# hbaatz/nerf-tex

Measured on AMD Instinct MI355X. Metric: ray-samples/sec (MLP+composite) at 800x800x64, higher is better.
Workload: dtype f32; 1 GPU; carpet 800x800x64: 640000 all-hit rays x 64 samples per GPU (BASELINE configs[1]), ParamNerf n_parameters=[1, 6], seeded glorot weights, inputs resident in HBM, fused PE+MLP+composite; rays_per_gpu=640000, hit_rays_total=640000, samples_per_ray=64

## Files before the change

nerf_tex_amd/csrc/ntx_backend_chain.hip:

```cpp
#include <algorithm>
#include <cstdio>
#include <cstdlib>
#include "ntx_trainer.h"
#include "ntx_train_device.h"
#include "ntx_encode.h"
namespace ntx_train {
enum { PACK_HIDDEN = 0, PACK_LINEAR = 1, PACK_AUX_ROW = 2, PACK_AUX_RGB = 3, PACK_COPY = 4 };
struct PackSeg {
    const float *src; long long sk, sc;
    int mode;
    int K, ncols, nt;
    float *dst; long long first, count;
};
struct PackArgs { const PackSeg *seg; int n_seg; long long total; };
__global__ void pack_kernel(PackArgs a) {
    const long long e = (long long)blockIdx.x * blockDim.x + threadIdx.x;
    if (e >= a.total) return;
    int lo = 0, hi = a.n_seg - 1;
    while (lo < hi) { const int mid = (lo + hi + 1) >> 1; if (a.seg[mid].first <= e) lo = mid; else hi = mid - 1; }
    const PackSeg &p = a.seg[lo];
    const long long o = e - p.first;
    float v = 0.0f;
    if (p.mode == PACK_COPY) v = p.src[o];
    else if (p.mode == PACK_AUX_ROW) {
        const int h = (int)(o >> 7) & 1, V = (int)(o & 127), k = hidden_row(V, h);
        v = k < p.K ? p.src[k * p.sk] : 0.0f;
    } else if (p.mode == PACK_AUX_RGB) {
        const int c = (int)(o >> 7), h = (int)(o >> 6) & 1, V = (int)(o & 63);
        v = p.src[hidden_row(V, h) * 3 + c];
    } else {
        const int c = (int)(o & 3), lane = (int)((o >> 2) & 63);
        const long long rec = o >> 8;
        const int G = p.nt / 4, g = (int)(rec % G), s = (int)(rec / G);
        const int f = lane & 31, kh = lane >> 5;
        const int k = p.mode == PACK_HIDDEN ? hidden_row(s, kh) : 2 * s + kh, col = 32 * (4 * g + c) + f;
        if (k < p.K && col < p.ncols) v = p.src[k * p.sk + col * p.sc];
    }
    p.dst[o] = v;
}

struct EncodeArgs {
    StepRays r;
    float *posO; int ptiles;
    float *dirO; int dtiles;
    float *dists;
};
template <bool IPE>
__global__ __launch_bounds__(64) void encode_kernel(EncodeArgs args) {
    const StepRays &a = args.r;
    const int lane = threadIdx.x, n = lane & 31, h = lane >> 5, blk = blockIdx.x, part = blockIdx.y;
    const long long m = (long long)blk * 32 + n;
    const bool valid = m < a.M();
    const int ray = valid ? (int)(m / a.S) : 0, s = valid ? (int)(m - (long long)ray * a.S) : 0;
    const int P = a.n_geo + a.n_app;
    const RayCtx rc = ray_ctx(a.rays_d, a.params, a.rays_per_param_row, ray, IPE ? P + 1 : P);
    const float *zray = a.z + (size_t)ray * (IPE ? a.S + 1 : a.S);
    const float e0 = zray[s], e1 = IPE ? zray[s + 1] : 0.0f;
    bool hit;
    const float z = depth_of(e0, hit);
    if (IPE) hit = hit && isfinite(e1);
    auto param = [&](int c) { return IPE ? spliced_param(rc.pr, c, a.blur_idx) : blurred_param(rc.pr, c, a.blur_idx, hit, a.cone, ray, z); };
    float *O = part == 0 ? args.posO : args.dirO;
    const int tiles = part == 0 ? args.ptiles : args.dtiles;
    auto put = [&](int row, float v) { O[o_index(blk, tiles, row, n)] = valid ? v : 0.0f; };
    auto fourier = [&](int r0, int D, int L, auto x) {
        if (h == 0) for (int c = 0; c < D; ++c) put(r0 + c, x(c));
        for (int f = 0; f < L; ++f)
            for (int c = 0; c < D; ++c) put(r0 + fourier_row_of(D, f, h, c), fourier_value(x(c), f, h));
    };
    if (part == 0) {
        int geo0;
        if (IPE) {
            float mean[3] = {a.rays_o[3 * ray], a.rays_o[3 * ray + 1], a.rays_o[3 * ray + 2]}, cov[3] = {0.0f, 0.0f, 0.0f};
            if (hit) {
                float t_mean, t_var, r_var;
                ntx::cone_moments((e0 + e1) / 2.0f, (e1 - e0) / 2.0f, rc.pr[a.blur_idx] * a.cone[ray], t_mean, t_var, r_var);
                for (int c = 0; c < 3; ++c) mean[c] = mean[c] + rc.d[c] * t_mean;
                ntx::cone_cov(t_var, r_var, rc.d, cov);
            }
            const int L = a.pos_freq;
            for (int f = 0; f < L; ++f)
                for (int c = 0; c < 3; ++c)
                    put(h * 3 * L + 3 * f + c, ntx::sin_q(mean[c] * ldexpf(1.0f, f), h) * expf(-0.5f * (cov[c] * ldexpf(1.0f, 2 * f))));
            geo0 = 6 * L;
        } else {
            const float o[3] = {a.rays_o[3 * ray], a.rays_o[3 * ray + 1], a.rays_o[3 * ray + 2]};
            fourier(0, 3, a.pos_freq, [&](int c) { return rc.point(o[c], c, z); });
            geo0 = fourier_width(3, a.pos_freq);
        }
        if (a.n_geo > 0) fourier(geo0, a.n_geo, a.param_freq, [&](int c) { return param(c); });
    } else {
        fourier(0, 3, a.dir_freq, [&](int c) { return rc.dir(c); });
        if (a.n_app > 0) fourier(fourier_width(3, a.dir_freq), a.n_app, a.param_freq, [&](int c) { return param(a.n_geo + c); });
        if (valid && h == 0) args.dists[(size_t)ray * a.S + s] = IPE ? segment_dist(e0, e1, hit, rc.dn) : sample_dist(zray, s, a.S, z, hit, rc.dn);
    }
}

struct EncodeSamplesArgs { StepSamples s; float *posO; int ptiles; float *dirO; int dtiles; };
__global__ __launch_bounds__(64) void encode_samples_kernel(EncodeSamplesArgs args) {
    const StepSamples &a = args.s;
    const int lane = threadIdx.x, n = lane & 31, h = lane >> 5, blk = blockIdx.x, part = blockIdx.y;
    const long long row = (long long)blk * 32 + n;
    const bool valid = row < a.n_live;
    const long long m = valid ? a.live[row] : 0, ray = m / a.S;
    const int P = a.n_geo + a.n_app;
    auto param = [&](int col) {
        if (!valid) return 0.0f;
        const float p = a.params_map[(size_t)m * P + col];
        return col == a.blur_idx ? p * a.blur_scale(m, ray) : p;
    };
    float *O = part == 0 ? args.posO : args.dirO;
    const int tiles = part == 0 ? args.ptiles : args.dtiles;
    auto put = [&](int r, float v) { O[o_index(blk, tiles, r, n)] = valid ? v : 0.0f; };
    auto fourier = [&](int r0, int D, int L, auto x) {
        if (h == 0) for (int c = 0; c < D; ++c) put(r0 + c, x(c));
        for (int f = 0; f < L; ++f)
            for (int c = 0; c < D; ++c) put(r0 + fourier_row_of(D, f, h, c), fourier_value(x(c), f, h));
    };
    const float *xyz = part == 0 ? a.pts : a.rays_d_map;
    const float x3[3] = {valid ? xyz[3 * m] : 0.0f, valid ? xyz[3 * m + 1] : 0.0f, valid ? xyz[3 * m + 2] : 0.0f};
    const int L3 = part == 0 ? a.pos_freq : a.dir_freq, D = part == 0 ? a.n_geo : a.n_app, c0 = part == 0 ? 0 : a.n_geo;
    fourier(0, 3, L3, [&](int c) { return c == 0 ? x3[0] : c == 1 ? x3[1] : x3[2]; });
    if (D > 0) fourier(fourier_width(3, L3), D, a.param_freq, [&](int c) { return param(c0 + c); });
}
__global__ __launch_bounds__(256) void dhead_rows_kernel(const float *__restrict__ dgrad, long long n_live, float *__restrict__ dhead) {
    const long long m = (long long)blockIdx.x * 256 + threadIdx.x;
    if (m >= (n_live + 31) / 32 * 32) return;
    const f32x4 zero = {0.0f, 0.0f, 0.0f, 0.0f};
    const f32x4 g = m < n_live ? *reinterpret_cast<const f32x4 *>(dgrad + 4 * m) : zero;
    dhead[o_index(m >> 5, 1, 0, (int)(m & 31))] = g.x; dhead[o_index(m >> 5, 1, 1, (int)(m & 31))] = g.y;
    dhead[o_index(m >> 5, 1, 2, (int)(m & 31))] = g.z; dhead[o_index(m >> 5, 1, 3, (int)(m & 31))] = g.w;
}

struct DirRowArgs {
    StepRays r; int Kd, splice;
    const float *w, *bias;
    float *rows;
};
__global__ __launch_bounds__(256) void dirrow_kernel(DirRowArgs a) {
    __shared__ float feat[8 * MAX_PB_GROUPS];
    const int ray = blockIdx.x, f = threadIdx.x;
    const RayCtx r = ray_ctx(a.r.rays_d, a.r.params, a.r.rays_per_param_row, ray, a.r.n_geo + a.r.n_app + (a.splice >= 0 ? 1 : 0));
    if (f < a.Kd) {
        const int K3 = fourier_width(3, a.r.dir_freq);
        const bool xyz = f < K3;
        feat[f] = fourier_row(xyz ? f : f - K3, xyz ? 3 : a.r.n_app, [&](int c) { return xyz ? r.dir(c) : spliced_param(r.pr, a.r.n_geo + c, a.splice); });
    }
    __syncthreads();
    float acc = a.bias[f];
    for (int k = 0; k < a.Kd; ++k) acc = fmaf(feat[k], a.w[(size_t)k * 256 + f], acc);
    const int T = f >> 5, g = (f >> 3) & 3, h = (f >> 2) & 1, c = f & 3;
    a.rows[(size_t)ray * 256 + h * 128 + 16 * T + 4 * g + c] = acc;
}

struct FeatGradArgs {
    const float *dY[2], *W[2]; int n_terms;
    int K, ld; long long M;
    float *G;
};
template <int NT>
__global__ __launch_bounds__(256) void feat_grad_kernel(FeatGradArgs a) {
    const int lane = threadIdx.x & 63, n = lane & 31, h = lane >> 5;
    const int wave = __builtin_amdgcn_readfirstlane(blockIdx.x * 4 + (threadIdx.x >> 6)), nwaves = gridDim.x * 4;
    const int n_blocks = (int)((a.M + 31) >> 5);
    const uint32_t voff_y = o_lane_bytes(lane);
    uint32_t voff_w[NT];
    static_for<NT>([&](auto T) { constexpr int t = T; voff_w[t] = (uint32_t)(32 * t + n) * 1024u + (uint32_t)h * 16u; });
    for (int blk = wave; blk < n_blocks; blk += nwaves) {
        f32x16 acc[NT];
        static_for<NT>([&](auto T) { acc[T] = f32x16{0.f, 0.f, 0.f, 0.f, 0.f, 0.f, 0.f, 0.f, 0.f, 0.f, 0.f, 0.f, 0.f, 0.f, 0.f, 0.f}; });
        for (int term = 0; term < a.n_terms; ++term) {
            const __amdgpu_buffer_rsrc_t rw = make_rsrc(a.W[term], (long long)a.K * 1024);
            const __amdgpu_buffer_rsrc_t ry = make_rsrc(a.dY[term] + (size_t)blk * 8 * 1024, 8 * 4096);
            f32x4 wa[2][4][NT]; float yb[2][16];
            auto fetch = [&](auto BUF, int grp) {
                constexpr int buf = BUF;
                static_for<4>([&](auto Q) {
                    constexpr int q = Q;
                    static_for<NT>([&](auto T) {
                        wa[buf][q][T] = __builtin_bit_cast(f32x4, __builtin_amdgcn_raw_buffer_load_b128(rw, voff_w[T], (uint32_t)(4 * grp + q) * 32u, 0)); });
                    static_for<4>([&](auto Cc) {
                        constexpr int c = Cc;
                        yb[buf][4 * q + c] = __builtin_bit_cast(float, __builtin_amdgcn_raw_buffer_load_b32(ry, voff_y, (uint32_t)grp * 4096u + o_value_bytes(4 * q + c), 0)); });
                });
            };
            auto compute = [&](auto BUF) {
                constexpr int buf = BUF;
                static_for<4>([&](auto Q) { static_for<4>([&](auto Cc) { static_for<NT>([&](auto T) {
                    constexpr int q = Q, c = Cc;
                    acc[T] = mfma32(wa[buf][q][T][c], yb[buf][4 * q + c], acc[T]);
                }); }); });
            };
            fetch(std::integral_constant<int, 0>{}, 0);
            for (int grp = 0; grp < 8; grp += 2) {
                fetch(std::integral_constant<int, 1>{}, grp + 1);
                compute(std::integral_constant<int, 0>{});
                fetch(std::integral_constant<int, 0>{}, grp + 2 < 8 ? grp + 2 : grp + 1);
                compute(std::integral_constant<int, 1>{});
            }
        }
        const long long m = (long long)blk * 32 + n;
        if (m < a.M) {
            float *row = a.G + (size_t)m * a.ld;
            static_for<NT>([&](auto T) { static_for<4>([&](auto Gq) {
                constexpr int t = T, g = Gq;
                const int j = 32 * t + 8 * g + 4 * h;
                if (j < a.ld) *reinterpret_cast<f32x4 *>(row + j) = f32x4{acc[t][4 * g], acc[t][4 * g + 1], acc[t][4 * g + 2], acc[t][4 * g + 3]};
            }); });
        }
    }
}

}
namespace {
using namespace ntx_train;
struct ChainBackend : Backend {
    ntx_trainer *t = nullptr;
    int ptiles = 0, dtiles = 0, PS = 0, DS = 0, fwd_variant = 0;
    TLayer trunk[8], feature, c1, c2, rgb, alpha;
    float *wfwd = nullptr, *wdx = nullptr, *aux = nullptr; size_t fwd_floats = 0, dx_floats = 0;
    PackSeg *pack_seg = nullptr; int n_pack = 0; long long pack_total = 0;
    float *posO = nullptr, *dirO = nullptr;
    float *act = nullptr; long long act_stride = 0;
    unsigned int *bits = nullptr; long long bits_stride = 0;
    float *dirrow = nullptr;
    float *gout = nullptr; long long gout_stride = 0;
    DwJob *jobs = nullptr; int n_jobs = 0; long long total_cost = 0;
    std::vector<DwJob> jobs_host; std::vector<int> reduce_job;
    float *dw_partial = nullptr; ReduceBatch reduce{};
    float *G_pos = nullptr, *G_dir = nullptr; int ld_pos = 0, ld_dir = 0;
    float *ray_pg = nullptr;
    float *act_at(int i) const { return act + (size_t)i * act_stride; }
    float *gout_at(int i) const { return gout + (size_t)i * gout_stride; }
    bool samples_on = false;
    static int blocks_of(long long rows) { return (int)((rows + 31) / 32); }
    unsigned chain_grid(long long rows) const { return (unsigned)std::min<long long>(t->cus, (blocks_of(rows) + 3) / 4); }
    unsigned feat_grid(long long rows) const { return (unsigned)std::min<long long>(2 * (long long)t->cus, (blocks_of(rows) + 3) / 4); }
    size_t plan_layers(const ntx_model_desc &d, bool ipe);
    void build_pack();
    void build_dw_jobs();
    int forward(const StepRays &r, hipStream_t st) override;
    int backward(const StepRays &r, hipStream_t st) override;
    void launch_pack(hipStream_t st);
    FwdArgs fwd_args(long long M) const;
    void backward_network(long long M, hipStream_t st);
    void backward_weights(int n_blocks, hipStream_t st);
    int takes_samples() override { return samples_on ? NTX_OK : Backend::takes_samples(); }
    int enable_samples() override;
    int forward_samples(const StepSamples &s, hipStream_t st) override;
    int backward_samples(const StepSamples &s, float *sample_pg, hipStream_t st) override;
    int enable_gradients(int param_mode, int input_mode) override;
    void launch_feat_grad(hipStream_t st, unsigned grid, int tiles, const FeatGradArgs &a);
    int activation(int layer, int64_t n_samples_total, float *out_host) override;
};

size_t ChainBackend::plan_layers(const ntx_model_desc &d, bool ipe) {
    const ntx::BlobView n = ntx::view_blob(ntx::tuned_arch(1), ntx::dims_of(&d), ipe);
    const int Kp = n.pos_map, Kd = n.dir_map;
    ptiles = (Kp + 31) / 32; dtiles = (Kd + 31) / 32;
    const int psg = ((Kp + 1) / 2 + 3) / 4, dsg = ((Kd + 1) / 2 + 3) / 4;
    fwd_variant = 3;
    for (int v = 2; v >= 0; --v)
        if (FWD_VARIANTS[v][0] >= psg && FWD_VARIANTS[v][1] >= dsg &&
            FWD_VARIANTS[v][0] + FWD_VARIANTS[v][1] <= FWD_VARIANTS[fwd_variant][0] + FWD_VARIANTS[fwd_variant][1]) fwd_variant = v;
    PS = 4 * FWD_VARIANTS[fwd_variant][0]; DS = 4 * FWD_VARIANTS[fwd_variant][1];
    std::copy(n.trunk.begin(), n.trunk.end(), trunk);
    feature = n.feature; c1 = n.colour[0]; c2 = n.c2; rgb = n.rgb; alpha = n.alpha;
    return n.count;
}

void ChainBackend::build_pack() {
    const int Kp = t->Kp, Kd = t->Kd;
    enum { FWD = 0, DX = 1, AUX = 2 };
    std::vector<PackSeg> segs; std::vector<int> base_of;
    size_t floats[2] = {0, 0};
    long long first = 0;
    auto push = [&](PackSeg s, int base, size_t at, long long count) {
        s.count = count; s.first = first; s.dst = (float *)(uintptr_t)(at * sizeof(float));
        first += count; segs.push_back(s); base_of.push_back(base);
    };
    auto seg = [&](const float *src, long long sk, long long sc, int mode, int K, int ncols, int nt, int stream, int nsteps) {
        PackSeg s{}; s.src = src; s.sk = sk; s.sc = sc; s.mode = mode; s.K = K; s.ncols = ncols; s.nt = nt;
        const int ring = stream == DX ? DX_RING : RING;
        const long long recs = ((long long)nsteps * (nt / 4) + ring - 1) / ring * ring;
        push(s, stream, floats[stream], recs * 256); floats[stream] += (size_t)recs * 256;
    };
    const float *W = t->w;
    auto fwd_hidden = [&](const TLayer &l, int row0, int nt) { seg(W + l.w + (size_t)row0 * l.out, l.out, 1, PACK_HIDDEN, 256, l.out, nt, FWD, 128); };
    auto fwd_linear = [&](const TLayer &l, int K, int nsteps) { seg(W + l.w, l.out, 1, PACK_LINEAR, K, l.out, 8, FWD, nsteps); };
    fwd_linear(trunk[0], Kp, PS);
    for (int i = 1; i < 8; ++i) {
        if (i == 5) { fwd_linear(trunk[5], Kp, PS); fwd_hidden(trunk[5], Kp, 8); }
        else fwd_hidden(trunk[i], 0, 8);
    }
    fwd_hidden(feature, 0, 8);
    fwd_linear(c1, Kd, DS); fwd_hidden(c1, Kd, 8);
    fwd_hidden(c2, 0, 4);
    const size_t n_fwd_segs = segs.size();
    auto dx_hidden = [&](const TLayer &l, int row0, int K, int nsteps) { seg(W + l.w + (size_t)row0 * l.out, 1, l.out, PACK_HIDDEN, K, 256, 8, DX, nsteps); };
    seg(W + rgb.w, 1, 3, PACK_LINEAR, 3, 128, 4, DX, 2);
    dx_hidden(c2, 0, 128, 64);
    dx_hidden(c1, Kd, 256, 128);
    dx_hidden(feature, 0, 256, 128);
    seg(W + alpha.w, 1, 1, PACK_LINEAR, 1, 256, 8, DX, 1);
    for (int i = 7; i >= 1; --i) dx_hidden(trunk[i], i == 5 ? Kp : 0, 256, 128);
    auto tail = [&](size_t of, int stream) { const long long count = (long long)(stream == DX ? DX_RING : RING) * 256; push(segs[of], stream, floats[stream], count); floats[stream] += (size_t)count; };
    tail(0, FWD); tail(n_fwd_segs, DX);
    auto aux_seg = [&](const float *src, int mode, int K, long long count, size_t at) { PackSeg s{}; s.src = src; s.sk = 1; s.mode = mode; s.K = K; push(s, AUX, at, count); };
    for (int i = 0; i < 8; ++i) aux_seg(W + trunk[i].b, PACK_AUX_ROW, 256, 256, AUX_BIAS + (size_t)i * 256);
    aux_seg(W + feature.b, PACK_AUX_ROW, 256, 256, AUX_BIAS + 8 * 256); aux_seg(W + c1.b, PACK_AUX_ROW, 256, 256, AUX_BIAS + 9 * 256);
    aux_seg(W + c2.b, PACK_AUX_ROW, 128, 256, AUX_BIAS + 10 * 256);
    aux_seg(W + alpha.w, PACK_AUX_ROW, 256, 256, AUX_ALPHA_W); aux_seg(W + alpha.b, PACK_COPY, 1, 1, AUX_ALPHA_B);
    aux_seg(W + rgb.w, PACK_AUX_RGB, 128, 384, AUX_RGB_W); aux_seg(W + rgb.b, PACK_COPY, 3, 3, AUX_RGB_B);
    pack_total = first; n_pack = (int)segs.size(); fwd_floats = floats[FWD]; dx_floats = floats[DX];
    t->mem.alloc(&wfwd, fwd_floats); t->mem.alloc(&wdx, dx_floats); t->mem.alloc(&aux, AUX_FLOATS, true);
    float *const base[3] = {wfwd, wdx, aux};
    for (size_t i = 0; i < segs.size(); ++i) segs[i].dst = (float *)((char *)base[base_of[i]] + (uintptr_t)segs[i].dst);
    t->mem.upload(&pack_seg, segs, "segment");
}

void ChainBackend::build_dw_jobs() {
    const int Kp = t->Kp, Kd = t->Kd;
    std::vector<DwJob> &jobs = jobs_host;
    struct RJ { int job; long long at, count, pair; size_t out; };
    std::vector<RJ> rjobs;
    auto new_job = [&]() { DwJob j{}; for (DwWave &w : j.w) w.shape = -1; jobs.push_back(j); return (int)jobs.size() - 1; };
    auto matrix = [&](int j, int K, int N, size_t g_kernel, long long g_bias, long long *at_bias) {
        const long long at = jobs[j].slot_floats;
        jobs[j].slot_floats += (long long)K * N;
        rjobs.push_back(RJ{j, at, (long long)K * N, 0, g_kernel});
        *at_bias = -1;
        if (g_bias >= 0) { *at_bias = jobs[j].slot_floats; jobs[j].slot_floats += 2 * N; rjobs.push_back(RJ{j, *at_bias, N, N, (size_t)g_bias}); }
        return at;
    };
    auto wave = [&](int j, int w, int shape, const float *A, int rtA, int a0, const float *B, int rtB, int b0, long long at, int K, int N, int c_lo, long long at_bias) {
        DwWave &d = jobs[j].w[w];
        d.A = A; d.rtA = rtA; d.a0 = a0; d.B = B; d.rtB = rtB; d.b0 = b0; d.shape = shape; d.out = at; d.ldc = N; d.row0 = a0 * 32; d.rows_valid = K;
        d.col0 = b0 * 32; d.c_lo = c_lo; d.c_hi = c_lo + N; d.bias_out = a0 == 0 ? at_bias : -1;
        const int cost = shape == 0 ? 256 : shape == 1 ? 198 : 68;
        if (cost > jobs[j].cost) jobs[j].cost = cost;
    };
    auto layer_job = [&](const float *X, const float *dY, size_t g_kernel, size_t g_bias) {
        const int j = new_job(); long long ab; const long long at = matrix(j, 256, 256, g_kernel, (long long)g_bias, &ab);
        for (int w = 0; w < 4; ++w) wave(j, w, 0, X, 8, 4 * (w >> 1), dY, 8, 4 * (w & 1), at, 256, 256, 0, ab);
    };
    for (int i = 7; i >= 1; --i) layer_job(act_at(i - 1), gout_at(10 - i), trunk[i].w + (size_t)(i == 5 ? Kp : 0) * 256, trunk[i].b);
    layer_job(act_at(7), gout_at(2), feature.w, feature.b);
    layer_job(act_at(8), gout_at(1), c1.w + (size_t)Kd * 256, c1.b);
    {
        const int j = new_job(); long long ab0, ab5;
        const long long at0 = matrix(j, Kp, 256, trunk[0].w, (long long)trunk[0].b, &ab0), at5 = matrix(j, Kp, 256, trunk[5].w, -1, &ab5);
        for (int w = 0; w < 2; ++w) { wave(j, w, 1, posO, ptiles, 0, gout_at(10), 8, 4 * w, at0, Kp, 256, 0, ab0); wave(j, 2 + w, 1, posO, ptiles, 0, gout_at(5), 8, 4 * w, at5, Kp, 256, 0, ab5); }
    }
    {
        const int j = new_job(); long long abd, ab2;
        const long long atd = matrix(j, Kd, 256, c1.w, -1, &abd), at2 = matrix(j, 256, 128, c2.w, (long long)c2.b, &ab2);
        for (int w = 0; w < 2; ++w) { wave(j, w, 1, dirO, dtiles, 0, gout_at(1), 8, 4 * w, atd, Kd, 256, 0, abd); wave(j, 2 + w, 0, act_at(9), 8, 4 * w, gout_at(0), 4, 0, at2, 256, 128, 0, ab2); }
    }
    {
        const int j = new_job(); long long abr, aba;
        const long long atr = matrix(j, 128, 3, rgb.w, (long long)rgb.b, &abr), ata = matrix(j, 256, 1, alpha.w, (long long)alpha.b, &aba);
        wave(j, 0, 2, act_at(10), 4, 0, t->dhead, 1, 0, atr, 128, 3, 0, abr);
        for (int w = 0; w < 2; ++w) wave(j, 1 + w, 2, act_at(7), 8, 4 * w, t->dhead, 1, 0, ata, 256, 1, 3, aba);
    }
    n_jobs = (int)jobs.size();
    size_t partial_floats = 0;
    for (DwJob &j : jobs) total_cost += j.cost;
    for (DwJob &j : jobs) {
        const long long slots = ((long long)j.cost * t->cus + total_cost - 1) / total_cost + 2;
        j.first_float = (long long)partial_floats; partial_floats += (size_t)(slots * j.slot_floats);
    }
    t->mem.alloc(&dw_partial, partial_floats);
    t->mem.upload(&this->jobs, jobs, "job");
    if (t->mem.rc == NTX_OK && (int)rjobs.size() > MAX_REDUCE_BATCH) t->mem.rc = ntx_set_error(NTX_E_INVALID, "trainer: too many weight gradients for one launch");
    long long rfirst = 0;
    for (size_t i = 0; i < rjobs.size() && t->mem.rc == NTX_OK; ++i) {
        ReduceJob &r = reduce.job[reduce.n++];
        const DwJob &j = jobs[rjobs[i].job];
        r.partial = dw_partial + j.first_float + rjobs[i].at; r.n_split = 0; r.stride = j.slot_floats; r.count = rjobs[i].count; r.pair = rjobs[i].pair;
        r.out = t->grad + rjobs[i].out; r.first = rfirst;
        rfirst += (rjobs[i].count + 255) / 256 * 256;
        reduce_job.push_back(rjobs[i].job);
    }
}

void ChainBackend::launch_pack(hipStream_t st) {
    const PackArgs pa{pack_seg, n_pack, pack_total};
    hipLaunchKernelGGL(pack_kernel, dim3((unsigned)((pack_total + 255) / 256)), dim3(256), 0, st, pa);
}
FwdArgs ChainBackend::fwd_args(long long M) const {
    FwdArgs f{}; f.stream = wfwd; f.stream_bytes = (uint32_t)(fwd_floats * sizeof(float)); f.aux = aux; f.M = M;
    f.ptiles = ptiles; f.dtiles = dtiles; f.pos = posO; f.dir = dirO;
    f.act = act; f.act_stride = act_stride; f.bits = bits; f.bits_stride = bits_stride;
    f.sigma = t->sigma; f.raw_rgb = t->raw_rgb;
    return f;
}
int ChainBackend::forward(const StepRays &r, hipStream_t st) {
    launch_pack(st);
    EncodeArgs e{}; e.r = r; e.posO = posO; e.ptiles = ptiles; e.dirO = dirO; e.dtiles = dtiles; e.dists = t->dists;
    if (t->ipe) hipLaunchKernelGGL(encode_kernel<true>, dim3((unsigned)r.n_blocks(), 2), dim3(64), 0, st, e);
    else hipLaunchKernelGGL(encode_kernel<false>, dim3((unsigned)r.n_blocks(), 2), dim3(64), 0, st, e);
    FwdArgs f = fwd_args(r.M());
    const bool hoist = (t->ipe || r.blur_idx < 0 || r.blur_idx < r.n_geo) && r.S % 32 == 0 && getenv("NERFTEX_TRAIN_NO_DIR_HOIST") == nullptr;
    if (hoist) {
        DirRowArgs dr{}; dr.r = r; dr.Kd = t->Kd; dr.w = t->w + c1.w; dr.bias = t->w + c1.b; dr.rows = dirrow; dr.splice = t->ipe ? r.blur_idx : -1;
        hipLaunchKernelGGL(dirrow_kernel, dim3((unsigned)r.n_rays), dim3(256), 0, st, dr);
    }
    f.dirrow = dirrow; f.n_rays = (int)r.n_rays; f.S = r.S;
    launch_fwd_chain(fwd_variant, hoist, st, chain_grid(r.M()), f);
    return NTX_OK;
}
int ChainBackend::forward_samples(const StepSamples &s, hipStream_t st) {
    if (int rc = takes_samples()) return rc;
    const long long M = s.n_live;
    if (M == 0) return NTX_OK;
    launch_pack(st);
    EncodeSamplesArgs e{}; e.s = s; e.posO = posO; e.ptiles = ptiles; e.dirO = dirO; e.dtiles = dtiles;
    hipLaunchKernelGGL(encode_samples_kernel, dim3((unsigned)blocks_of(M), 2), dim3(64), 0, st, e);
    FwdArgs f = fwd_args(M);
    f.dirrow = dirrow; f.n_rays = (int)s.n_rays; f.S = s.S;
    launch_fwd_chain(fwd_variant, false, st, chain_grid(M), f);
    return NTX_OK;
}

#ifdef NTX_TRAIN_CLOCKS
unsigned long long *dw_clocks_buffer(long long G, int n_jobs, hipStream_t st) {
    static unsigned long long *clocks = nullptr;
    const size_t nck = (size_t)G * (2 + 3 * n_jobs);
    if (!getenv("NERFTEX_DW_CLOCKS")) return nullptr;
    if (!clocks) (void)hipMalloc((void **)&clocks, nck * sizeof(unsigned long long));
    (void)hipMemsetAsync(clocks, 0, nck * sizeof(unsigned long long), st);
    return clocks;
}
void dump_dw_clocks(const unsigned long long *clocks, long long G, const std::vector<DwJob> &jobs, hipStream_t st) {
    const int n_jobs = (int)jobs.size();
    const size_t nck = (size_t)G * (2 + 3 * n_jobs);
    std::vector<unsigned long long> h(nck);
    (void)hipStreamSynchronize(st);
    (void)hipMemcpy(h.data(), clocks, nck * sizeof(unsigned long long), hipMemcpyDeviceToHost);
    unsigned long long t0 = ~0ull;
    for (long long g = 0; g < G; ++g) t0 = std::min(t0, h[g * (2 + 3 * n_jobs)]);
    FILE *f = fopen(getenv("NERFTEX_DW_CLOCKS"), "w");
    if (!f) return;
    for (long long g = 0; g < G; ++g) {
        const unsigned long long *c = &h[g * (2 + 3 * n_jobs)];
        fprintf(f, "%lld %llu %llu", g, c[0] - t0, c[1] - t0);
        for (int j = 0; j < n_jobs; ++j) if (c[4 + 3 * j]) fprintf(f, "  j%d cost %d blocks %llu %llu-%llu", j, jobs[j].cost, c[2 + 3 * j], c[3 + 3 * j] - t0, c[4 + 3 * j] - t0);
        fprintf(f, "\n");
    }
    fclose(f);
}
#endif

void ChainBackend::backward_network(long long M, hipStream_t st) {
    DxArgs x{}; x.stream = wdx; x.stream_bytes = (uint32_t)(dx_floats * sizeof(float)); x.M = M; x.dgrad = t->dgrad;
    x.out = gout; x.out_stride = gout_stride; x.bits = bits; x.bits_stride = bits_stride;
    launch_dx_chain(st, chain_grid(M), x);
    if (t->pg_mode != 0 || t->ig_mode != 0) {
        FeatGradArgs p{}; p.dY[0] = gout_at(10); p.W[0] = t->w + trunk[0].w; p.dY[1] = gout_at(5); p.W[1] = t->w + trunk[5].w; p.n_terms = 2;
        p.K = t->Kp; p.ld = ld_pos; p.M = M; p.G = G_pos;
        launch_feat_grad(st, feat_grid(M), ptiles, p);
        FeatGradArgs d{}; d.dY[0] = gout_at(1); d.W[0] = t->w + c1.w; d.n_terms = 1; d.K = t->Kd; d.ld = ld_dir; d.M = M; d.G = G_dir;
        launch_feat_grad(st, feat_grid(M), dtiles, d);
    }
    if (t->takes_weight_gradients()) backward_weights(blocks_of(M), st);
}
int ChainBackend::backward(const StepRays &r, hipStream_t st) {
    backward_network(r.M(), st);
    if (t->pg_mode != 0) {
        const ntx_model_desc &m = t->desc;
        launch_param_fold(st, r, G_pos + 3 * (1 + 2 * m.pos_freq), G_dir + 3 * (1 + 2 * m.dir_freq), ld_pos, ld_dir, ray_pg, t->P, t->param_grad);
    }
    if (t->ig_mode != 0) launch_ray_fold(st, r, G_pos, G_dir, ld_pos, ld_dir, t->dgrad, t->sigma, t->step_noise, t->d_rays_o, t->d_rays_d);
    return NTX_OK;
}
int ChainBackend::backward_samples(const StepSamples &s, float *sample_pg, hipStream_t st) {
    if (int rc = takes_samples()) return rc;
    const long long M = s.n_live;
    if (M > 0) {
        hipLaunchKernelGGL(dhead_rows_kernel, dim3((unsigned)((blocks_of(M) * 32 + 255) / 256)), dim3(256), 0, st, t->dgrad, M, t->dhead);
        backward_network(M, st);
    } else if (t->takes_weight_gradients()) TRAIN_TRY(hipMemsetAsync(t->grad, 0, t->n_weights * sizeof(float), st));
    const ntx_model_desc &m = t->desc;
    if (t->pg_mode != 0) launch_param_samples(st, s, G_pos + 3 * (1 + 2 * m.pos_freq), G_dir + 3 * (1 + 2 * m.dir_freq), ld_pos, ld_dir, t->P, sample_pg);
    if (t->ig_mode != 0) launch_input_samples(st, s, G_pos, G_dir, ld_pos, ld_dir, t->d_pts, t->d_dirs);
    return NTX_OK;
}
int ChainBackend::enable_samples() {
    if (t->ipe) return ntx_set_error(NTX_E_UNSUPPORTED, "an instanced step of an IPE model: the instanced render has no cone segments (out of scope, as on the layer-by-layer trainer)");
    if (samples_on) return NTX_OK;
    TRAIN_TRY(hipSetDevice(t->device));
    if (int rc = t->place_sample_maps()) return rc;
    samples_on = true;
    return NTX_OK;
}
void ChainBackend::backward_weights(int n_blocks, hipStream_t st) {
    DwArgs d{}; d.jobs = jobs; d.n_jobs = n_jobs; d.n_blocks = n_blocks; d.total_cost = total_cost; d.partial = dw_partial;
    const long long G = t->cus, W = total_cost * n_blocks;
#ifdef NTX_TRAIN_CLOCKS
    d.clocks = dw_clocks_buffer(G, n_jobs, st);
#endif
    launch_dw(st, (unsigned)G, d);
#ifdef NTX_TRAIN_CLOCKS
    if (d.clocks) dump_dw_clocks(d.clocks, G, jobs_host, st);
#endif
    ReduceBatch rb = reduce;
    std::vector<int> slots(n_jobs);
    long long start = 0;
    for (int j = 0; j < n_jobs; ++j) {
        const long long span = (long long)jobs_host[j].cost * n_blocks;
        slots[j] = (int)(dw_last_g(G, W, start, span) - dw_first_g(G, W, start) + 1);
        start += span;
    }
    for (int i = 0; i < rb.n; ++i) rb.job[i].n_split = slots[reduce_job[i]];
    launch_reduce(st, rb);
}

void ChainBackend::launch_feat_grad(hipStream_t st, unsigned grid, int tiles, const FeatGradArgs &a) {
    if (tiles <= 1) hipLaunchKernelGGL(feat_grad_kernel<1>, dim3(grid), dim3(256), 0, st, a);
    else if (tiles == 2) hipLaunchKernelGGL(feat_grad_kernel<2>, dim3(grid), dim3(256), 0, st, a);
    else hipLaunchKernelGGL(feat_grad_kernel<3>, dim3(grid), dim3(256), 0, st, a);
}

int ChainBackend::enable_gradients(int param_mode, int input_mode) {
    if (param_mode == 0 && input_mode == 0) return NTX_OK;
    if (t->ipe) return ntx_set_error(NTX_E_UNSUPPORTED, "parameter / input gradients of an IPE model on the fused chain: the cone gaussians' derivative is not written");
    if (G_pos) return NTX_OK;
    DeviceMemory &mem = t->mem;
    TRAIN_TRY(hipSetDevice(t->device));
    ld_pos = pad4(t->Kp); ld_dir = pad4(t->Kd);
    mem.alloc(&G_dir, (size_t)t->cap * ld_dir);
    mem.alloc(&ray_pg, (size_t)t->cap_rays * t->P); mem.alloc(&t->param_grad, (size_t)t->cap_rays * t->P);
    mem.alloc(&t->d_rays_o, (size_t)t->cap_rays * 3); mem.alloc(&t->d_rays_d, (size_t)t->cap_rays * 3);
    mem.alloc(&G_pos, (size_t)t->cap * ld_pos);
    return mem.rc;
}

int ChainBackend::activation(int layer, int64_t n_samples_total, float *out_host) {
    const float *src = nullptr; int tiles = 8;
    if (layer >= 0 && layer < 8) src = act_at(layer);
    else if (layer == 8) src = act_at(9);
    else if (layer == 9) { src = act_at(10); tiles = 4; }
    else if (layer == 10) src = t->sigma;
    else if (layer >= 20 && layer < 28) src = gout_at(10 - (layer - 20));
    else if (layer == 28) src = gout_at(1);
    else if (layer == 29) src = gout_at(2);
    else if (layer == 11) src = t->raw_rgb;
    else if (layer == 30) src = t->dgrad;
    else if ((layer == 40 || layer == 41) && G_pos && ((t->pg_mode != 0 && (t->pg_rows > 0 || t->spg_rays > 0)) || (t->ig_mode != 0 && (t->ig_rays > 0 || t->ig_smp_rays > 0)))) src = layer == 40 ? G_pos : G_dir;
    else return ntx_set_error(NTX_E_INVALID, "layer %d (0-7 trunk, 8 / 9 the colour layers, 10 the density, 11 the raw colour; 20-29 the kept gradients, 30 the composite's adjoint; "
                              "40 / 41 the gradient at pos_map / dir_map of a step under ntx_trainer_enable_gradients)", layer);
    TRAIN_TRY(hipSetDevice(t->device));
    TRAIN_TRY(hipDeviceSynchronize());
    if (layer == 40 || layer == 41) {
        const int K = layer == 40 ? t->Kp : t->Kd, ld = layer == 40 ? ld_pos : ld_dir;
        TRAIN_TRY(hipMemcpy2D(out_host, (size_t)K * sizeof(float), src, (size_t)ld * sizeof(float), (size_t)K * sizeof(float), (size_t)n_samples_total, hipMemcpyDeviceToHost));
        return NTX_OK;
    }
    if (layer == 10 || layer == 11 || layer == 30) {
        const size_t width = layer == 10 ? 1 : (layer == 11 ? 3 : 4);
        TRAIN_TRY(hipMemcpy(out_host, src, (size_t)n_samples_total * width * sizeof(float), hipMemcpyDeviceToHost)); return NTX_OK;
    }
    const long long nb = (n_samples_total + 31) / 32;
    std::vector<float> tmp((size_t)nb * tiles * 1024);
    TRAIN_TRY(hipMemcpy(tmp.data(), src, tmp.size() * sizeof(float), hipMemcpyDeviceToHost));
    const int width = tiles * 32;
    for (long long m = 0; m < n_samples_total; ++m)
        for (int row = 0; row < width; ++row) out_host[(size_t)m * width + row] = tmp[o_index(m >> 5, tiles, row, (int)(m & 31))];
    return NTX_OK;
}
}
namespace ntx_train {
template <int K, bool HOIST> void launch_fwd_variant(hipStream_t st, unsigned grid, const FwdArgs &a);
void launch_fwd_chain(int variant, bool hoist, hipStream_t st, unsigned grid, const FwdArgs &a) {
    static void (*const launch[8])(hipStream_t, unsigned, const FwdArgs &) = {launch_fwd_variant<0, false>, launch_fwd_variant<0, true>, launch_fwd_variant<1, false>, launch_fwd_variant<1, true>,
                                                                               launch_fwd_variant<2, false>, launch_fwd_variant<2, true>, launch_fwd_variant<3, false>, launch_fwd_variant<3, true>};
    launch[variant * 2 + (hoist ? 1 : 0)](st, grid, a);
}

int chain_check(const ntx_model_desc *desc, TrainDims *dims) {
    const bool ipe = desc->pos_encoding == NTX_POS_IPE && desc->n_pos == 6;
    if (desc->kind != NTX_MODEL_PARAMNERF || desc->depth != 8 || desc->width != 256 || desc->skip != 4 || desc->color_depth != 1 ||
        !((desc->pos_encoding == NTX_POS_FOURIER && desc->n_pos == 3) || ipe))
        return ntx_set_error(NTX_E_UNSUPPORTED, "training is built for the ParamNerf architecture of the shipped training configs (depth 8, width 256, skips [4], color_depth 1, "
                                                "Fourier features on n_pos 3 or IPE on n_pos 6); other architectures train through ntx_trainer_create_flex");
    if (desc->n_geo < 0 || desc->n_app < 0 || desc->n_geo + desc->n_app > 16) return ntx_set_error(NTX_E_INVALID, "n_parameters out of range");
    if (desc->pos_freq < 0 || desc->dir_freq < 0 || desc->param_freq < 0) return ntx_set_error(NTX_E_INVALID, "negative band count");
    const int Kp = ntx::pos_map_m(ntx::dims_of(desc), ipe), Kd = ntx::dir_map_m(ntx::dims_of(desc));
    if (Kp > 8 * MAX_PB_GROUPS || Kd > 8 * MAX_PB_GROUPS)
        return ntx_set_error(NTX_E_UNSUPPORTED, "training: pos_map (%d) / dir_map (%d) wider than %d features (the chain holds a block's encoded inputs in registers)", Kp, Kd,
                             8 * MAX_PB_GROUPS);
    dims->desc = *desc; dims->Kp = Kp; dims->Kd = Kd; dims->ipe = ipe; dims->n_weights = ChainBackend().plan_layers(*desc, ipe);
    return NTX_OK;
}

int chain_backend_create(ntx_trainer *t) {
    ChainBackend *c = new ChainBackend();
    t->backend = c; c->t = t;
    c->plan_layers(t->desc, t->ipe);
    DeviceMemory &mem = t->mem;
    const long long NB = t->cap_blocks;
    mem.alloc(&c->posO, (size_t)NB * c->ptiles * 1024, true); mem.alloc(&c->dirO, (size_t)NB * c->dtiles * 1024, true);
    c->act_stride = c->gout_stride = NB * 8 * 1024; c->bits_stride = NB * 256;
    mem.alloc(&c->act, (size_t)c->act_stride * 11); mem.alloc(&c->bits, (size_t)c->bits_stride * 10); mem.alloc(&c->gout, (size_t)c->gout_stride * 11);
    mem.alloc(&c->dirrow, (size_t)t->cap_rays * 256);
    c->build_pack();
    c->build_dw_jobs();
    return mem.rc;
}
}
```

nerf_tex_amd/csrc/ntx_train_device.h:

```cpp
#pragma once

#include "ntx_device.h"

namespace ntx_train {

using ntx::f32x16;
using ntx::f32x4;
using ntx::hidden_row;
using ntx::mfma32;
using ntx::RING;
using ntx::static_for;
typedef float f32x2 __attribute__((ext_vector_type(2)));
typedef int i32x4 __attribute__((ext_vector_type(4)));
typedef unsigned int u32x4 __attribute__((ext_vector_type(4)));

#define TRN_DEV __device__ __forceinline__

TRN_DEV __amdgpu_buffer_rsrc_t make_rsrc(const void *base, long long bytes) {
    const long long b = bytes < 0 ? 0 : (bytes > 0x7ffffff0ll ? 0x7ffffff0ll : bytes);
    return __builtin_amdgcn_make_buffer_rsrc(const_cast<void *>(base), 0, (int)b, 0x00020000);
}

TRN_DEV uint32_t o_lane_bytes(int lane) {
    const int n = lane & 31, h = lane >> 5;
    return (uint32_t)((n >> 3) * 1024 + ((n >> 2) & 1) * 512 + h * 64 + (n & 3) * 4);
}
constexpr int STORE_NT = 0;
constexpr uint32_t o_value_bytes(int V) { return (uint32_t)((V >> 4) * 4096 + ((V & 15) >> 2) * 128 + (V & 3) * 16); }

template <int R>
struct WRingT {
    static constexpr int DEPTH = R;
    __amdgpu_buffer_rsrc_t rsrc;
    uint32_t voff;
    f32x4 r[R];
};
typedef WRingT<RING> WRing;
constexpr int DX_RING = 16;
template <class WR>
TRN_DEV f32x4 wr_load(const WR &w, uint32_t byte_off) {
#ifdef NTX_X_WSMALL
    byte_off &= 0xffffu;
#endif
#ifdef NTX_X_NOWLOAD
    if (byte_off >= (uint32_t)WR::DEPTH * 1024u) return w.r[(byte_off >> 10) % WR::DEPTH];
#endif
    return __builtin_bit_cast(f32x4, __builtin_amdgcn_raw_buffer_load_b128(w.rsrc, w.voff, byte_off, 0));
}

template <int NSTEPS, int NMT, bool ZERO, class WR, class Extra>
TRN_DEV void seg_hidden(f32x16 (&acc)[8], WR &ws, uint32_t &sbase, const float (&hin)[128], Extra &&extra) {
    constexpr int RPS = NMT / 4, RING = WR::DEPTH;
    static_assert((NSTEPS * RPS) % RING == 0, "whole ring turns");
    const f32x16 zero = {0.f, 0.f, 0.f, 0.f, 0.f, 0.f, 0.f, 0.f, 0.f, 0.f, 0.f, 0.f, 0.f, 0.f, 0.f, 0.f};
    static_for<NSTEPS>([&](auto S) {
        constexpr int s = S;
        f32x4 w;
        static_for<NMT>([&](auto MT) {
            constexpr int mt = MT;
            if constexpr (mt % 4 == 0) {
                constexpr int rec = s * RPS + mt / 4;
                w = ws.r[rec % RING];
                ws.r[rec % RING] = wr_load(ws, sbase + (uint32_t)(rec + RING) * 1024u);
            }
            if constexpr (ZERO && s == 0) acc[mt] = mfma32(w[mt % 4], hin[s], zero);
            else acc[mt] = mfma32(w[mt % 4], hin[s], acc[mt]);
            extra(S, MT);
            __builtin_amdgcn_sched_barrier(0);
        });
    });
    sbase += (uint32_t)(NSTEPS * RPS) * 1024u;
}

template <int NG, class Fetch>
TRN_DEV void seg_mem(f32x16 (&acc)[8], WRing &ws, uint32_t &sbase, float (&pb)[12], Fetch &&fetch) {
    static_assert(RING == 8, "a group of 4 k-steps of 8 tiles is one ring turn");
    static_for<NG>([&](auto G) {
        constexpr int g = G;
        if constexpr (g + 2 < NG) fetch(std::integral_constant<int, g + 2>{});
        static_for<4>([&](auto K) {
            constexpr int k = K;
            f32x4 w;
            static_for<8>([&](auto MT) {
                constexpr int mt = MT;
                if constexpr (mt % 4 == 0) {
                    constexpr int slot = 2 * k + mt / 4;
                    w = ws.r[slot];
                    ws.r[slot] = wr_load(ws, sbase + (uint32_t)(8 * g + slot + RING) * 1024u);
                }
                acc[mt] = mfma32(w[mt % 4], pb[4 * (g % 3) + k], acc[mt]);
                __builtin_amdgcn_sched_barrier(0);
            });
        });
    });
    sbase += (uint32_t)NG * 8192u;
}

template <int NKS, int NMT, bool ZERO, class WR>
TRN_DEV void seg_few(f32x16 (&acc)[8], WR &ws, uint32_t &sbase, const float (&b)[NKS]) {
    constexpr int RPS = NMT / 4, RING = WR::DEPTH;
    static_assert(NKS * RPS <= RING, "one ring turn");
    const f32x16 zero = {0.f, 0.f, 0.f, 0.f, 0.f, 0.f, 0.f, 0.f, 0.f, 0.f, 0.f, 0.f, 0.f, 0.f, 0.f, 0.f};
    static_for<RING>([&](auto I) {
        constexpr int rec = I;
        const f32x4 w = ws.r[rec];
        ws.r[rec] = wr_load(ws, sbase + (uint32_t)(rec + RING) * 1024u);
        if constexpr (rec < NKS * RPS) {
            constexpr int s = rec / RPS, t0 = 4 * (rec % RPS);
            static_for<4>([&](auto C) {
                constexpr int c = C;
                if constexpr (ZERO && s == 0) acc[t0 + c] = mfma32(w[c], b[s], zero);
                else acc[t0 + c] = mfma32(w[c], b[s], acc[t0 + c]);
                __builtin_amdgcn_sched_barrier(0);
            });
        }
    });
    sbase += (uint32_t)RING * 1024u;
}

template <int V0>
TRN_DEV void convert8_relu_bits(float (&hin)[128], const f32x16 (&prev)[8], uint32_t &w) {
    constexpr int T = V0 >> 4, R = V0 & 15;
    float t0, t1, t2, t3;
    asm("v_accvgpr_read_b32 %0, %13\n\tv_accvgpr_read_b32 %1, %14\n\tv_accvgpr_read_b32 %2, %15\n\tv_accvgpr_read_b32 %3, %16\n\t"
        "v_accvgpr_read_b32 %4, %17\n\tv_accvgpr_read_b32 %5, %18\n\tv_accvgpr_read_b32 %6, %19\n\tv_accvgpr_read_b32 %7, %20\n\t"
        "v_sub_f32 %9, 0, %0\n\tv_sub_f32 %10, 0, %1\n\tv_sub_f32 %11, 0, %2\n\tv_sub_f32 %12, 0, %3\n\t"
        "v_alignbit_b32 %8, %8, %9, 31\n\tv_alignbit_b32 %8, %8, %10, 31\n\tv_alignbit_b32 %8, %8, %11, 31\n\tv_alignbit_b32 %8, %8, %12, 31\n\t"
        "v_sub_f32 %9, 0, %4\n\tv_sub_f32 %10, 0, %5\n\tv_sub_f32 %11, 0, %6\n\tv_sub_f32 %12, 0, %7\n\t"
        "v_alignbit_b32 %8, %8, %9, 31\n\tv_alignbit_b32 %8, %8, %10, 31\n\tv_alignbit_b32 %8, %8, %11, 31\n\tv_alignbit_b32 %8, %8, %12, 31\n\t"
        "v_max_f32 %0, 0, %0\n\tv_max_f32 %1, 0, %1\n\tv_max_f32 %2, 0, %2\n\tv_max_f32 %3, 0, %3\n\t"
        "v_max_f32 %4, 0, %4\n\tv_max_f32 %5, 0, %5\n\tv_max_f32 %6, 0, %6\n\tv_max_f32 %7, 0, %7"
        : "=&v"(hin[V0 + 0]), "=&v"(hin[V0 + 1]), "=&v"(hin[V0 + 2]), "=&v"(hin[V0 + 3]), "=&v"(hin[V0 + 4]), "=&v"(hin[V0 + 5]), "=&v"(hin[V0 + 6]),
          "=&v"(hin[V0 + 7]), "+v"(w), "=&v"(t0), "=&v"(t1), "=&v"(t2), "=&v"(t3)
        : "a"(prev[T][R + 0]), "a"(prev[T][R + 1]), "a"(prev[T][R + 2]), "a"(prev[T][R + 3]), "a"(prev[T][R + 4]), "a"(prev[T][R + 5]), "a"(prev[T][R + 6]),
          "a"(prev[T][R + 7]));
}
constexpr int keep_bit(int V) { return 31 - (V & 31); }

template <int NMT>
TRN_DEV void convert_relu_bits(float (&hin)[128], const f32x16 (&prev)[8], u32x4 &bits) {
    static_for<(NMT + 1) / 2>([&](auto W) {
        constexpr int wd = W;
        uint32_t w = 0;
        static_for<(NMT - 2 * wd >= 2 ? 4 : 2)>([&](auto Q) { convert8_relu_bits<32 * wd + 8 * decltype(Q)::value>(hin, prev, w); });
        bits[wd] = w;
    });
}
template <int NMT>
TRN_DEV void convert_linear(float (&hin)[128], const f32x16 (&prev)[8]) {
    static_for<NMT * 16>([&](auto V) { constexpr int v = V; hin[v] = prev[v >> 4][v & 15]; });
}
template <int NMT>
TRN_DEV void convert_mask(float (&hin)[128], const f32x16 (&prev)[8], const u32x4 &bits) {
    static_for<NMT * 16>([&](auto V) {
        constexpr int v = V;
        const float x = prev[v >> 4][v & 15];
        const int keep = __builtin_amdgcn_sbfe((int)bits[v >> 5], keep_bit(v), 1);
        hin[v] = __builtin_bit_cast(float, __builtin_bit_cast(int, x) & keep);
    });
}

constexpr int AUX_BIAS = 0, AUX_ALPHA_W = 11 * 256, AUX_ALPHA_B = AUX_ALPHA_W + 256, AUX_RGB_W = AUX_ALPHA_B + 4, AUX_RGB_B = AUX_RGB_W + 384,
              AUX_FLOATS = AUX_RGB_B + 4;
template <int MT>
TRN_DEV void bias_tile(f32x16 (&acc)[8], const float *aux, int layer, int h) {
    const f32x4 *b = reinterpret_cast<const f32x4 *>(aux + AUX_BIAS + layer * 256 + h * 128) + MT * 4;
    const f32x4 v0 = b[0], v1 = b[1], v2 = b[2], v3 = b[3];
    acc[MT] = f32x16{v0.x, v0.y, v0.z, v0.w, v1.x, v1.y, v1.z, v1.w, v2.x, v2.y, v2.z, v2.w, v3.x, v3.y, v3.z, v3.w};
}

constexpr int MAX_PB_GROUPS = 12;
struct FwdArgs {
    const float *stream; uint32_t stream_bytes;
    const float *aux;
    long long M;
    int ptiles, dtiles;
    const float *pos, *dir;
    float *act; long long act_stride;
    unsigned int *bits; long long bits_stride;
    float *sigma, *raw_rgb;
    const float *dirrow; int n_rays, S;
};

#ifdef NTX_TRAIN_FWD
template <int PSG, int DSG, bool HOIST>
__global__ __launch_bounds__(256) __attribute__((amdgpu_waves_per_eu(1, 1))) void fwd_chain_kernel(FwdArgs a) {
    __shared__ __attribute__((aligned(16))) float aux_lds[AUX_FLOATS];
    __shared__ __attribute__((aligned(16))) float rows_lds[HOIST ? 4 * 256 : 4];
    ntx::load_aux(aux_lds, a.aux, AUX_FLOATS);
    const int lane = threadIdx.x & 63, n = lane & 31, h = lane >> 5;
    const int wave = __builtin_amdgcn_readfirstlane(blockIdx.x * 4 + (threadIdx.x >> 6)), nwaves = gridDim.x * 4;
    const int n_blocks = (int)((a.M + 31) >> 5);
    if (wave >= n_blocks) return;
    WRing ws;
    ws.rsrc = make_rsrc(a.stream, a.stream_bytes);
    ws.voff = (uint32_t)lane * 16u;
    static_for<RING>([&](auto I) { ws.r[I] = wr_load(ws, (uint32_t)decltype(I)::value * 1024u); });
    const uint32_t lane_o = o_lane_bytes(lane), lane_r = (uint32_t)((n >> 3) * 1024 + ((n >> 2) & 1) * 512 + (n & 3) * 4 + h * 16), lane16 = (uint32_t)lane * 16u;
    float pb[12];
    const __amdgpu_buffer_rsrc_t rs_row = make_rsrc(a.dirrow, HOIST ? (long long)a.n_rays * 1024 : 0);
    __amdgpu_buffer_rsrc_t rs_in = make_rsrc(a.pos + (size_t)wave * a.ptiles * 1024, (long long)a.ptiles * 4096);
    auto fetch = [&](auto G) {
        constexpr int g = G;
        static_for<4>([&](auto K) {
            constexpr int k = K;
            constexpr int s = 4 * g + k;
            pb[4 * (g % 3) + k] = __builtin_bit_cast(float, __builtin_amdgcn_raw_buffer_load_b32(rs_in, lane_r, (uint32_t)((s >> 4) * 4096 + (s & 15) * 32), 0));
        });
    };
    fetch(std::integral_constant<int, 0>{}); fetch(std::integral_constant<int, 1>{});
    for (int blk = wave; blk < n_blocks; blk += nwaves) {
        uint32_t opaque_zero = 0;
        asm volatile("" : "+v"(opaque_zero));
        const float *aux = aux_lds + opaque_zero;
        const float *rows_aux = rows_lds + opaque_zero + (HOIST ? (threadIdx.x >> 6) * 256 : 0) - AUX_BIAS - 9 * 256;
        uint32_t sbase = 0;
        f32x16 acc[8];
        float hin[128];
        const long long m = (long long)blk * 32 + n;
        const bool valid = m < a.M;
        if constexpr (HOIST) {
            const uint32_t ray = __builtin_amdgcn_readfirstlane((int)(((uint32_t)blk * 32u) / (uint32_t)a.S));
            const f32x4 x0 = __builtin_bit_cast(f32x4, __builtin_amdgcn_raw_buffer_load_b128(rs_row, lane16, (ray < (uint32_t)a.n_rays ? ray : (uint32_t)a.n_rays - 1u) * 1024u, 0));
            *reinterpret_cast<f32x4 *>(rows_lds + (threadIdx.x >> 6) * 256 + lane * 4) = x0;
            __builtin_amdgcn_wave_barrier();
        }
        __amdgpu_buffer_rsrc_t rs_out = make_rsrc(a.act, 0);
        auto leaves_to = [&](int idx, int tiles) { rs_out = make_rsrc(a.act + (size_t)idx * a.act_stride + (size_t)blk * tiles * 1024, (long long)tiles * 4096); };
        auto leave = [&](auto V) {
            constexpr int v = V;
#ifndef NTX_X_NOSTORE
            __builtin_amdgcn_raw_buffer_store_b32(__builtin_bit_cast(int, hin[v]), rs_out, lane_o, o_value_bytes(v), STORE_NT);
#endif
        };
        auto bits_leave = [&](int idx, const u32x4 &bw) {
#ifndef NTX_X_NOBITS
            const __amdgpu_buffer_rsrc_t rb = make_rsrc(a.bits + (size_t)idx * a.bits_stride + (size_t)blk * 256, 1024);
            __builtin_amdgcn_raw_buffer_store_b128(__builtin_bit_cast(i32x4, bw), rb, lane16, 0, 0);
#endif
        };
        static_for<8>([&](auto T) { bias_tile<decltype(T)::value>(acc, aux, 0, h); });
        seg_mem<PSG>(acc, ws, sbase, pb, fetch);
        float sig_part = 0.0f;
        auto layer = [&](auto LIc) {
            f32x16 (&cur)[8] = acc; f32x16 (&prev)[8] = acc;
            constexpr int LI = decltype(LIc)::value, in_idx = LI - 1;
            constexpr bool relu_in = in_idx != 8;
            u32x4 bw = {0u, 0u, 0u, 0u};
            if constexpr (HOIST && LI == 9) {
                sbase += (uint32_t)DSG * 8192u;
                static_for<RING>([&](auto I) { ws.r[I] = wr_load(ws, sbase + (uint32_t)decltype(I)::value * 1024u); });
            }
            static_for<4>([&](auto W) {
                constexpr int wd = W;
                if constexpr (relu_in) {
                    uint32_t w = 0;
                    static_for<4>([&](auto Q) { convert8_relu_bits<32 * wd + 8 * decltype(Q)::value>(hin, prev, w); });
                    bw[wd] = w;
                } else static_for<32>([&](auto V) { constexpr int v = 32 * wd + decltype(V)::value; hin[v] = prev[v >> 4][v & 15]; });
                const float *bsrc = (HOIST && LI == 9) ? rows_aux : aux;
                if constexpr (LI < 10 || wd < 2) { bias_tile<2 * wd>(cur, bsrc, LI, h); bias_tile<2 * wd + 1>(cur, bsrc, LI, h); }
            });
            if constexpr (relu_in) bits_leave(in_idx < 8 ? in_idx : 8, bw);
            if constexpr (LI == 8) {
                const f32x4 *wa = reinterpret_cast<const f32x4 *>(aux + AUX_ALPHA_W + h * 128);
                static_for<32>([&](auto I) {
                    constexpr int i = I;
                    const f32x4 w = wa[i];
                    sig_part = __builtin_fmaf(hin[4 * i + 0], w.x, sig_part); sig_part = __builtin_fmaf(hin[4 * i + 1], w.y, sig_part);
                    sig_part = __builtin_fmaf(hin[4 * i + 2], w.z, sig_part); sig_part = __builtin_fmaf(hin[4 * i + 3], w.w, sig_part);
                });
            }
            __builtin_amdgcn_sched_barrier(0);
            leaves_to(in_idx, 8);
            if constexpr (LI == 5) seg_mem<PSG>(cur, ws, sbase, pb, fetch);
            if constexpr (LI == 9 && !HOIST) seg_mem<DSG>(cur, ws, sbase, pb, fetch);
            if constexpr (LI == 4) rs_in = make_rsrc(a.pos + (size_t)blk * a.ptiles * 1024, (long long)a.ptiles * 4096);
            if constexpr (LI == 8 && !HOIST) rs_in = make_rsrc(a.dir + (size_t)blk * a.dtiles * 1024, (long long)a.dtiles * 4096);
            if constexpr (LI == 10) {
                const int nb = blk + nwaves < n_blocks ? blk + nwaves : blk;
                rs_in = make_rsrc(a.pos + (size_t)nb * a.ptiles * 1024, (long long)a.ptiles * 4096);
            }
            auto extra = [&](auto S, auto MT) {
                constexpr int s = decltype(S)::value, mt = decltype(MT)::value;
                if constexpr ((LI == 4 || (LI == 8 && !HOIST) || LI == 10) && mt == 2 && (s == 8 || s == 24)) fetch(std::integral_constant<int, (s == 8 ? 0 : 1)>{});
                if constexpr (mt == 5 || (LI == 10 && mt == 3)) leave(S);
            };
            if constexpr (LI == 10) seg_hidden<128, 4, false>(cur, ws, sbase, hin, extra);
            else seg_hidden<128, 8, false>(cur, ws, sbase, hin, extra);
        };
        static_for<10>([&](auto I) { layer(std::integral_constant<int, decltype(I)::value + 1>{}); });
        {
            u32x4 bw = {0u, 0u, 0u, 0u};
            convert_relu_bits<4>(hin, acc, bw);
            bits_leave(9, bw);
            leaves_to(10, 4);
            static_for<64>([&](auto V) { leave(V); });
            float rgb[3];
            static_for<3>([&](auto C) {
                constexpr int c = C;
                const f32x4 *wc = reinterpret_cast<const f32x4 *>(aux + AUX_RGB_W + (c * 2 + h) * 64);
                float p = 0.0f;
                static_for<16>([&](auto I) {
                    constexpr int i = I;
                    const f32x4 w = wc[i];
                    p = __builtin_fmaf(hin[4 * i + 0], w.x, p); p = __builtin_fmaf(hin[4 * i + 1], w.y, p);
                    p = __builtin_fmaf(hin[4 * i + 2], w.z, p); p = __builtin_fmaf(hin[4 * i + 3], w.w, p);
                });
                rgb[c] = p + __shfl_xor(p, 32, 64) + aux[AUX_RGB_B + c];
            });
            const float sigma = sig_part + __shfl_xor(sig_part, 32, 64) + aux[AUX_ALPHA_B];
            if (valid && h == 0) {
                a.sigma[m] = sigma;
                a.raw_rgb[3 * m + 0] = rgb[0]; a.raw_rgb[3 * m + 1] = rgb[1]; a.raw_rgb[3 * m + 2] = rgb[2];
            }
        }
    }
}

#endif

struct DxArgs {
    const float *stream; uint32_t stream_bytes;
    long long M;
    const float *dgrad;
    float *out; long long out_stride;
    const unsigned int *bits; long long bits_stride;
};

#ifdef NTX_TRAIN_DX
__global__ __launch_bounds__(256) __attribute__((amdgpu_waves_per_eu(1, 1))) void dx_chain_kernel(DxArgs a) {
    const int lane = threadIdx.x & 63, n = lane & 31, h = lane >> 5;
    const int wave = __builtin_amdgcn_readfirstlane(blockIdx.x * 4 + (threadIdx.x >> 6)), nwaves = gridDim.x * 4;
    const int n_blocks = (int)((a.M + 31) >> 5);
    if (wave >= n_blocks) return;
    WRingT<DX_RING> ws;
    ws.rsrc = make_rsrc(a.stream, a.stream_bytes);
    ws.voff = (uint32_t)lane * 16u;
    static_for<DX_RING>([&](auto I) { ws.r[I] = wr_load(ws, (uint32_t)decltype(I)::value * 1024u); });
    const uint32_t lane_o = o_lane_bytes(lane), lane16 = (uint32_t)lane * 16u;
    auto fetch_grad = [&](int blk) {
        const long long m = (long long)blk * 32 + n;
        const f32x4 zero = {0.0f, 0.0f, 0.0f, 0.0f};
        return m < a.M ? *reinterpret_cast<const f32x4 *>(a.dgrad + 4 * m) : zero;
    };
    f32x4 g = fetch_grad(wave);
    for (int blk = wave; blk < n_blocks; blk += nwaves) {
        uint32_t sbase = 0;
        f32x16 acc[8];
        float hin[128];
        __amdgpu_buffer_rsrc_t rs_out = make_rsrc(a.out, 0);
        auto leaves_to = [&](int idx, int tiles) { rs_out = make_rsrc(a.out + (size_t)idx * a.out_stride + (size_t)blk * tiles * 1024, (long long)tiles * 4096); };
        auto leave = [&](auto V) {
            constexpr int v = V;
            __builtin_amdgcn_raw_buffer_store_b32(__builtin_bit_cast(int, hin[v]), rs_out, lane_o, o_value_bytes(v), STORE_NT);
        };
        auto fetch_bits = [&](int idx) {
            const __amdgpu_buffer_rsrc_t rb = make_rsrc(a.bits + (size_t)idx * a.bits_stride + (size_t)blk * 256, 1024);
            return __builtin_bit_cast(u32x4, __builtin_amdgcn_raw_buffer_load_b128(rb, lane16, 0, 0));
        };
        u32x4 bw = fetch_bits(9);
        const float gs = h ? 0.0f : g.w;
        {
            const float b[2] = {h ? g.y : g.x, h ? 0.0f : g.z};
            seg_few<2, 4, true>(acc, ws, sbase, b);
        }
        {
            const int nb = blk + nwaves < n_blocks ? blk + nwaves : blk;
            g = fetch_grad(nb);
        }
        convert_mask<4>(hin, acc, bw);
        bw = fetch_bits(8);
        leaves_to(0, 4);
        seg_hidden<64, 8, true>(acc, ws, sbase, hin, [&](auto S, auto MT) { if constexpr (decltype(MT)::value == 5) leave(S); });
        convert_mask<8>(hin, acc, bw);
        leaves_to(1, 8);
        seg_hidden<128, 8, true>(acc, ws, sbase, hin, [&](auto S, auto MT) { if constexpr (decltype(MT)::value == 5) leave(S); });
        convert_linear<8>(hin, acc);
        static_for<8>([&](auto J) {
            constexpr int j = J;
            bw = fetch_bits(7 - j);
            leaves_to(2 + j, 8);
            seg_hidden<128, 8, true>(acc, ws, sbase, hin, [&](auto S, auto MT) { if constexpr (decltype(MT)::value == 5) leave(S); });
            if constexpr (j == 0) {
                const float b[1] = {gs};
                seg_few<1, 8, false>(acc, ws, sbase, b);
            }
            convert_mask<8>(hin, acc, bw);
        });
        leaves_to(10, 8);
        static_for<128>([&](auto V) { leave(V); });
    }
}

#endif

struct DwWave {
    const float *A; int rtA, a0;
    const float *B; int rtB, b0;
    int shape;
    long long out; int ldc;
    int row0, rows_valid, col0, c_lo, c_hi;
    long long bias_out;
};
struct DwJob { DwWave w[4]; int cost; long long slot_floats, first_float; };
struct DwArgs { const DwJob *jobs; int n_jobs, n_blocks; long long total_cost; float *partial;
                unsigned long long *clocks; };

__host__ __device__ inline long long dw_cut(long long g, long long G, long long W, long long start, long long cost, long long n_blocks) {
    const long long x = g * W / G - start;
    long long b = x <= 0 ? 0 : (x + cost / 2) / cost;
    return b > n_blocks ? n_blocks : b;
}
__host__ __device__ inline long long dw_first_g(long long G, long long W, long long start) { return start * G / W; }
__host__ __device__ inline long long dw_last_g(long long G, long long W, long long start, long long span) { return (start + span - 1) * G / W; }

#ifdef NTX_TRAIN_DW
#ifndef NTX_DW_SYNC
#define NTX_DW_SYNC 16
#endif
constexpr int DW_SYNC = NTX_DW_SYNC;
template <int NA, int NB>
TRN_DEV void dw_piece(const DwWave &tg, float *slot, int blk0, int blk1, int lane) {
    auto uniform_ptr = [](const float *p) {
        const uint32_t lo = (uint32_t)__builtin_amdgcn_readfirstlane((int)(uint32_t)(uintptr_t)p), hi = (uint32_t)__builtin_amdgcn_readfirstlane((int)(uint32_t)((uintptr_t)p >> 32));
        return (const float *)(uintptr_t)(((uint64_t)hi << 32) | (uint64_t)lo);
    };
    const float *A = uniform_ptr(tg.A), *B = uniform_ptr(tg.B);
    const int rtA = __builtin_amdgcn_readfirstlane(tg.rtA), a0 = __builtin_amdgcn_readfirstlane(tg.a0), rtB = __builtin_amdgcn_readfirstlane(tg.rtB), b0 = __builtin_amdgcn_readfirstlane(tg.b0);
    f32x16 acc[NA][NB];
    static_for<NA>([&](auto Ai) { static_for<NB>([&](auto Bi) {
        acc[Ai][Bi] = f32x16{0.f, 0.f, 0.f, 0.f, 0.f, 0.f, 0.f, 0.f, 0.f, 0.f, 0.f, 0.f, 0.f, 0.f, 0.f, 0.f}; }); });
    f32x4 bsum[NB];
    static_for<NB>([&](auto Bi) { bsum[Bi] = f32x4{0.0f, 0.0f, 0.0f, 0.0f}; });
    const bool want_bias = tg.bias_out >= 0;
    const int nblk = blk1 - blk0;
    if (nblk > 0) {
        const __amdgpu_buffer_rsrc_t ra = make_rsrc(A + (size_t)blk0 * rtA * 1024, (long long)nblk * rtA * 4096);
        const __amdgpu_buffer_rsrc_t rb = make_rsrc(B + (size_t)blk0 * rtB * 1024, (long long)nblk * rtB * 4096);
        const uint32_t voff = (uint32_t)lane * 16u;
        const uint32_t stepA = (uint32_t)rtA * 4096u, stepB = (uint32_t)rtB * 4096u, offA = (uint32_t)a0 * 4096u, offB = (uint32_t)b0 * 4096u;
        f32x4 xa[2][NA][2], xb[2][NB][2];
        auto fetch = [&](auto BUF, int i) {
            constexpr int buf = BUF;
#ifdef NTX_X_DWSMALL
            i &= 3;
#endif
#ifdef NTX_X_DWNOLOAD
            if (i > 0) return;
#endif
            const uint32_t oa = (uint32_t)i * stepA + offA + (uint32_t)buf * 2048u, ob = (uint32_t)i * stepB + offB + (uint32_t)buf * 2048u;
            static_for<NA>([&](auto Ai) { static_for<2>([&](auto Q) {
                xa[buf][Ai][Q] = __builtin_bit_cast(f32x4, __builtin_amdgcn_raw_buffer_load_b128(ra, voff, oa + (uint32_t)(decltype(Ai)::value * 4 + decltype(Q)::value) * 1024u, 0)); }); });
            static_for<NB>([&](auto Bi) { static_for<2>([&](auto Q) {
                xb[buf][Bi][Q] = __builtin_bit_cast(f32x4, __builtin_amdgcn_raw_buffer_load_b128(rb, voff, ob + (uint32_t)(decltype(Bi)::value * 4 + decltype(Q)::value) * 1024u, 0)); }); });
        };
        auto compute = [&](auto BUF) {
            constexpr int buf = BUF;
            static_for<2>([&](auto Q) { static_for<4>([&](auto C) {
                constexpr int q = Q, c = C;
                static_for<NA>([&](auto Ai) { static_for<NB>([&](auto Bi) {
                    acc[Ai][Bi] = mfma32(xa[buf][Ai][q][c], xb[buf][Bi][q][c], acc[Ai][Bi]);
                }); });
            }); });
            if (want_bias) static_for<NB>([&](auto Bi) { bsum[Bi] += xb[buf][Bi][0] + xb[buf][Bi][1]; });
        };
        fetch(std::integral_constant<int, 0>{}, 0);
        for (int i = 0; i < nblk; ++i) {
            if ((i & (DW_SYNC - 1)) == 0) __builtin_amdgcn_s_barrier();
            fetch(std::integral_constant<int, 1>{}, i);
            __builtin_amdgcn_sched_barrier(0);
            compute(std::integral_constant<int, 0>{});
            __builtin_amdgcn_sched_barrier(0);
            fetch(std::integral_constant<int, 0>{}, i + 1 < nblk ? i + 1 : i);
            __builtin_amdgcn_sched_barrier(0);
            compute(std::integral_constant<int, 1>{});
            __builtin_amdgcn_sched_barrier(0);
        }
    }
    const int j = lane & 31, hh = lane >> 5;
    const int ldc = __builtin_amdgcn_readfirstlane(tg.ldc), row0 = __builtin_amdgcn_readfirstlane(tg.row0), rows_valid = __builtin_amdgcn_readfirstlane(tg.rows_valid);
    const int col0 = __builtin_amdgcn_readfirstlane(tg.col0), c_lo = __builtin_amdgcn_readfirstlane(tg.c_lo), c_hi = __builtin_amdgcn_readfirstlane(tg.c_hi);
    const long long at_out = (long long)(((uint64_t)(uint32_t)__builtin_amdgcn_readfirstlane((int)(uint32_t)((uint64_t)tg.out >> 32)) << 32) | (uint32_t)__builtin_amdgcn_readfirstlane((int)(uint32_t)(uint64_t)tg.out));
    const __amdgpu_buffer_rsrc_t ro = make_rsrc(slot + at_out, (long long)rows_valid * ldc * 4);
    constexpr uint32_t NOWHERE = 0x7ffffff0u;
    static_for<NB>([&](auto Bi) {
        const int col = col0 + 32 * decltype(Bi)::value + j;
        const bool col_ok = col >= c_lo && col < c_hi;
        const uint32_t coff = (uint32_t)(col - c_lo) * 4u;
        static_for<NA>([&](auto Ai) {
            static_for<16>([&](auto R) {
                constexpr int r = R;
                const int row = row0 + 32 * decltype(Ai)::value + 8 * (r >> 2) + (r & 3) + 4 * hh;
                const uint32_t off = (col_ok && row < rows_valid) ? (uint32_t)(row * ldc) * 4u + coff : NOWHERE;
                __builtin_amdgcn_raw_buffer_store_b32(__builtin_bit_cast(int, (float)acc[Ai][Bi][r]), ro, off, 0, 0);
            });
        });
    });
    if (want_bias) {
        const long long at_bias = (long long)(((uint64_t)(uint32_t)__builtin_amdgcn_readfirstlane((int)(uint32_t)((uint64_t)tg.bias_out >> 32)) << 32) | (uint32_t)__builtin_amdgcn_readfirstlane((int)(uint32_t)(uint64_t)tg.bias_out));
        float *bo = slot + at_bias + (size_t)hh * (c_hi - c_lo);
        static_for<NB>([&](auto Bi) {
            const int col = col0 + 32 * decltype(Bi)::value + j;
            const f32x4 sm = bsum[Bi];
            if (col >= c_lo && col < c_hi) bo[col - c_lo] = (sm.x + sm.y) + (sm.z + sm.w);
        });
    }
}

__global__ __launch_bounds__(256) __attribute__((amdgpu_waves_per_eu(1, 1))) void dw_kernel(DwArgs a) {
    const int lane = threadIdx.x & 63, wave = __builtin_amdgcn_readfirstlane(threadIdx.x >> 6);
    const long long g = blockIdx.x, G = gridDim.x, W = a.total_cost * a.n_blocks;
    long long start = 0;
#ifdef NTX_TRAIN_CLOCKS
    unsigned long long *ck = a.clocks ? a.clocks + (size_t)blockIdx.x * (2 + 3 * a.n_jobs) : nullptr;
    if (ck && threadIdx.x == 0) ck[0] = wall_clock64();
#endif
    for (int jn = 0; jn < a.n_jobs; ++jn) {
        const DwJob &job = a.jobs[jn];
        const long long cost = job.cost, span = cost * a.n_blocks;
        const long long g0 = dw_first_g(G, W, start), g1 = dw_last_g(G, W, start, span);
        if (__builtin_amdgcn_readfirstlane((int)(g >= g0 && g <= g1))) {
            const int blk0 = __builtin_amdgcn_readfirstlane((int)dw_cut(g, G, W, start, cost, a.n_blocks)), blk1 = __builtin_amdgcn_readfirstlane((int)dw_cut(g + 1, G, W, start, cost, a.n_blocks));
            const DwWave &wv = job.w[wave];
            const int shape = __builtin_amdgcn_readfirstlane(wv.shape);
            const int my_slot = __builtin_amdgcn_readfirstlane((int)(g - g0));
            float *slot = a.partial + job.first_float + (long long)my_slot * job.slot_floats;
#ifdef NTX_TRAIN_CLOCKS
            const unsigned long long c0 = wall_clock64();
#endif
            if (shape == 0) dw_piece<4, 4>(wv, slot, blk0, blk1, lane);
            else if (shape == 1) dw_piece<3, 4>(wv, slot, blk0, blk1, lane);
            else if (shape == 2) dw_piece<4, 1>(wv, slot, blk0, blk1, lane);
            else for (int i = 0; i < blk1 - blk0; i += DW_SYNC) __builtin_amdgcn_s_barrier();
#ifdef NTX_TRAIN_CLOCKS
            __syncthreads();
            if (ck && threadIdx.x == 0) { ck[2 + 3 * jn] = (unsigned long long)(blk1 - blk0); ck[3 + 3 * jn] = c0; ck[4 + 3 * jn] = wall_clock64(); }
#endif
        }
        start += span;
    }
#ifdef NTX_TRAIN_CLOCKS
    if (ck && threadIdx.x == 0) ck[1] = wall_clock64();
#endif
}
#endif

constexpr int FWD_VARIANTS[4][2] = {{9, 11}, {9, 8}, {11, 8}, {MAX_PB_GROUPS, MAX_PB_GROUPS}};
void launch_fwd_chain(int variant, bool hoist, hipStream_t st, unsigned grid, const FwdArgs &a);
void launch_dx_chain(hipStream_t st, unsigned grid, const DxArgs &a);
void launch_dw(hipStream_t st, unsigned grid, const DwArgs &a);

}
```

Measured before the change: 112.4 million ray-samples/s.

## Fold linear feature layer into c1 weights to drop one 256x256 GEMM

The feature layer has no activation, so its weights are multiplied into the hidden part of the c1 weights (with a combined bias) by a small fold kernel before packing. The forward and dx chains then run one fewer 256x256 layer per sample. The weight-gradient path computes the gradient of the folded matrix and unfolds it into separate feature and c1 gradients. The feature-gradient debug output is rebuilt on request. This adds small fold/unfold kernels per step and changes floating-point rounding order.

After: 112.2 million ray-samples/s. Within noise of the previous version (-0.1%).

```diff
diff --git a/nerf_tex_amd/csrc/ntx_backend_chain.hip b/nerf_tex_amd/csrc/ntx_backend_chain.hip
--- a/nerf_tex_amd/csrc/ntx_backend_chain.hip
+++ b/nerf_tex_amd/csrc/ntx_backend_chain.hip
@@ -37,6 +37,51 @@
         if (k < p.K && col < p.ncols) v = p.src[k * p.sk + col * p.sc];
     }
     p.dst[o] = v;
+}
+
+struct FoldProduct {
+    const float *A; int ai, ap; const float *B; int bp, bj; float *C;
+    const float *u, *v;
+    const float *arow, *cadd; float *crow;
+    float *arow_copy;
+};
+struct FoldArgs { FoldProduct p[2]; };
+__global__ __launch_bounds__(256) void fold_kernel(FoldArgs args) {
+    __shared__ float As[32][33], Bs[32][33];
+    const FoldProduct &q = args.p[blockIdx.z];
+    const bool rides = blockIdx.y == 8;
+    if (rides && !q.crow) return;
+    const int tx = threadIdx.x & 31, ty = threadIdx.x >> 5, i0 = blockIdx.y * 32, j0 = blockIdx.x * 32;
+    float acc[4] = {0.0f, 0.0f, 0.0f, 0.0f};
+    for (int p0 = 0; p0 < 256; p0 += 32) {
+        for (int r = ty; r < 32; r += 8) {
+            As[r][tx] = rides ? (r == 0 ? q.arow[p0 + tx] : 0.0f) : q.A[(size_t)(i0 + r) * q.ai + (size_t)(p0 + tx) * q.ap];
+            Bs[r][tx] = q.B[(size_t)(p0 + r) * q.bp + (size_t)(j0 + tx) * q.bj];
+        }
+        __syncthreads();
+        for (int p = 0; p < 32; ++p)
+            for (int k = 0; k < 4; ++k) acc[k] = fmaf(As[ty + 8 * k][p], Bs[p][tx], acc[k]);
+        __syncthreads();
+    }
+    if (rides) {
+        if (ty == 0) {
+            q.crow[j0 + tx] = q.cadd ? acc[0] + q.cadd[j0 + tx] : acc[0];
+            if (q.arow_copy) q.arow_copy[j0 + tx] = q.arow[j0 + tx];
+        }
+        return;
+    }
+    for (int k = 0; k < 4; ++k) {
+        const int i = i0 + ty + 8 * k;
+        q.C[(size_t)i * 256 + j0 + tx] = q.u ? fmaf(q.u[i], q.v[j0 + tx], acc[k]) : acc[k];
+    }
+}
+__global__ __launch_bounds__(256) void dfeature_kernel(const float *__restrict__ dc1, const float *__restrict__ w_c1f, float *__restrict__ out) {
+    const int blk = blockIdx.x, k = threadIdx.x;
+    for (int n = 0; n < 32; ++n) {
+        float acc = 0.0f;
+        for (int c = 0; c < 256; ++c) acc = fmaf(dc1[o_index(blk, 8, c, n)], w_c1f[(size_t)k * 256 + c], acc);
+        out[o_index(blk, 8, k, n)] = acc;
+    }
 }
 
 struct EncodeArgs {
@@ -220,6 +265,8 @@
     TLayer trunk[8], feature, c1, c2, rgb, alpha;
     float *wfwd = nullptr, *wdx = nullptr, *aux = nullptr; size_t fwd_floats = 0, dx_floats = 0;
     PackSeg *pack_seg = nullptr; int n_pack = 0; long long pack_total = 0;
+    float *fold = nullptr, *dfold = nullptr;
+    enum { FOLD_BIAS = 256 * 256, FOLD_FLOATS = 256 * 256 + 256 };
     float *posO = nullptr, *dirO = nullptr;
     float *act = nullptr; long long act_stride = 0;
     unsigned int *bits = nullptr; long long bits_stride = 0;
@@ -242,6 +289,7 @@
     int forward(const StepRays &r, hipStream_t st) override;
     int backward(const StepRays &r, hipStream_t st) override;
     void launch_pack(hipStream_t st);
+    void launch_unfold(hipStream_t st);
     FwdArgs fwd_args(long long M) const;
     void backward_network(long long M, hipStream_t st);
     void backward_weights(int n_blocks, hipStream_t st);
@@ -293,23 +341,22 @@
         if (i == 5) { fwd_linear(trunk[5], Kp, PS); fwd_hidden(trunk[5], Kp, 8); }
         else fwd_hidden(trunk[i], 0, 8);
     }
-    fwd_hidden(feature, 0, 8);
-    fwd_linear(c1, Kd, DS); fwd_hidden(c1, Kd, 8);
+    fwd_linear(c1, Kd, DS);
+    seg(fold, 256, 1, PACK_HIDDEN, 256, 256, 8, FWD, 128);
     fwd_hidden(c2, 0, 4);
     const size_t n_fwd_segs = segs.size();
     auto dx_hidden = [&](const TLayer &l, int row0, int K, int nsteps) { seg(W + l.w + (size_t)row0 * l.out, 1, l.out, PACK_HIDDEN, K, 256, 8, DX, nsteps); };
     seg(W + rgb.w, 1, 3, PACK_LINEAR, 3, 128, 4, DX, 2);
     dx_hidden(c2, 0, 128, 64);
-    dx_hidden(c1, Kd, 256, 128);
-    dx_hidden(feature, 0, 256, 128);
+    seg(fold, 1, 256, PACK_HIDDEN, 256, 256, 8, DX, 128);
     seg(W + alpha.w, 1, 1, PACK_LINEAR, 1, 256, 8, DX, 1);
     for (int i = 7; i >= 1; --i) dx_hidden(trunk[i], i == 5 ? Kp : 0, 256, 128);
     auto tail = [&](size_t of, int stream) { const long long count = (long long)(stream == DX ? DX_RING : RING) * 256; push(segs[of], stream, floats[stream], count); floats[stream] += (size_t)count; };
     tail(0, FWD); tail(n_fwd_segs, DX);
     auto aux_seg = [&](const float *src, int mode, int K, long long count, size_t at) { PackSeg s{}; s.src = src; s.sk = 1; s.mode = mode; s.K = K; push(s, AUX, at, count); };
     for (int i = 0; i < 8; ++i) aux_seg(W + trunk[i].b, PACK_AUX_ROW, 256, 256, AUX_BIAS + (size_t)i * 256);
-    aux_seg(W + feature.b, PACK_AUX_ROW, 256, 256, AUX_BIAS + 8 * 256); aux_seg(W + c1.b, PACK_AUX_ROW, 256, 256, AUX_BIAS + 9 * 256);
-    aux_seg(W + c2.b, PACK_AUX_ROW, 128, 256, AUX_BIAS + 10 * 256);
+    aux_seg(fold + FOLD_BIAS, PACK_AUX_ROW, 256, 256, AUX_BIAS + 8 * 256);
+    aux_seg(W + c2.b, PACK_AUX_ROW, 128, 256, AUX_BIAS + 9 * 256);
     aux_seg(W + alpha.w, PACK_AUX_ROW, 256, 256, AUX_ALPHA_W); aux_seg(W + alpha.b, PACK_COPY, 1, 1, AUX_ALPHA_B);
     aux_seg(W + rgb.w, PACK_AUX_RGB, 128, 384, AUX_RGB_W); aux_seg(W + rgb.b, PACK_COPY, 3, 3, AUX_RGB_B);
     pack_total = first; n_pack = (int)segs.size(); fwd_floats = floats[FWD]; dx_floats = floats[DX];
@@ -322,15 +369,15 @@
 void ChainBackend::build_dw_jobs() {
     const int Kp = t->Kp, Kd = t->Kd;
     std::vector<DwJob> &jobs = jobs_host;
-    struct RJ { int job; long long at, count, pair; size_t out; };
+    struct RJ { int job; long long at, count, pair; float *out; };
     std::vector<RJ> rjobs;
     auto new_job = [&]() { DwJob j{}; for (DwWave &w : j.w) w.shape = -1; jobs.push_back(j); return (int)jobs.size() - 1; };
-    auto matrix = [&](int j, int K, int N, size_t g_kernel, long long g_bias, long long *at_bias) {
+    auto matrix = [&](int j, int K, int N, float *g_kernel, float *g_bias, long long *at_bias) {
         const long long at = jobs[j].slot_floats;
         jobs[j].slot_floats += (long long)K * N;
         rjobs.push_back(RJ{j, at, (long long)K * N, 0, g_kernel});
         *at_bias = -1;
-        if (g_bias >= 0) { *at_bias = jobs[j].slot_floats; jobs[j].slot_floats += 2 * N; rjobs.push_back(RJ{j, *at_bias, N, N, (size_t)g_bias}); }
+        if (g_bias) { *at_bias = jobs[j].slot_floats; jobs[j].slot_floats += 2 * N; rjobs.push_back(RJ{j, *at_bias, N, N, g_bias}); }
         return at;
     };
     auto wave = [&](int j, int w, int shape, const float *A, int rtA, int a0, const float *B, int rtB, int b0, long long at, int K, int N, int c_lo, long long at_bias) {
@@ -340,27 +387,27 @@
         const int cost = shape == 0 ? 256 : shape == 1 ? 198 : 68;
         if (cost > jobs[j].cost) jobs[j].cost = cost;
     };
-    auto layer_job = [&](const float *X, const float *dY, size_t g_kernel, size_t g_bias) {
-        const int j = new_job(); long long ab; const long long at = matrix(j, 256, 256, g_kernel, (long long)g_bias, &ab);
+    auto layer_job = [&](const float *X, const float *dY, float *g_kernel, float *g_bias) {
+        const int j = new_job(); long long ab; const long long at = matrix(j, 256, 256, g_kernel, g_bias, &ab);
         for (int w = 0; w < 4; ++w) wave(j, w, 0, X, 8, 4 * (w >> 1), dY, 8, 4 * (w & 1), at, 256, 256, 0, ab);
     };
-    for (int i = 7; i >= 1; --i) layer_job(act_at(i - 1), gout_at(10 - i), trunk[i].w + (size_t)(i == 5 ? Kp : 0) * 256, trunk[i].b);
-    layer_job(act_at(7), gout_at(2), feature.w, feature.b);
-    layer_job(act_at(8), gout_at(1), c1.w + (size_t)Kd * 256, c1.b);
+    float *const G = t->grad;
+    for (int i = 7; i >= 1; --i) layer_job(act_at(i - 1), gout_at(9 - i), G + trunk[i].w + (size_t)(i == 5 ? Kp : 0) * 256, G + trunk[i].b);
+    layer_job(act_at(7), gout_at(1), dfold, dfold + FOLD_BIAS);
     {
         const int j = new_job(); long long ab0, ab5;
-        const long long at0 = matrix(j, Kp, 256, trunk[0].w, (long long)trunk[0].b, &ab0), at5 = matrix(j, Kp, 256, trunk[5].w, -1, &ab5);
-        for (int w = 0; w < 2; ++w) { wave(j, w, 1, posO, ptiles, 0, gout_at(10), 8, 4 * w, at0, Kp, 256, 0, ab0); wave(j, 2 + w, 1, posO, ptiles, 0, gout_at(5), 8, 4 * w, at5, Kp, 256, 0, ab5); }
+        const long long at0 = matrix(j, Kp, 256, G + trunk[0].w, G + trunk[0].b, &ab0), at5 = matrix(j, Kp, 256, G + trunk[5].w, nullptr, &ab5);
+        for (int w = 0; w < 2; ++w) { wave(j, w, 1, posO, ptiles, 0, gout_at(9), 8, 4 * w, at0, Kp, 256, 0, ab0); wave(j, 2 + w, 1, posO, ptiles, 0, gout_at(4), 8, 4 * w, at5, Kp, 256, 0, ab5); }
     }
     {
         const int j = new_job(); long long abd, ab2;
-        const long long atd = matrix(j, Kd, 256, c1.w, -1, &abd), at2 = matrix(j, 256, 128, c2.w, (long long)c2.b, &ab2);
-        for (int w = 0; w < 2; ++w) { wave(j, w, 1, dirO, dtiles, 0, gout_at(1), 8, 4 * w, atd, Kd, 256, 0, abd); wave(j, 2 + w, 0, act_at(9), 8, 4 * w, gout_at(0), 4, 0, at2, 256, 128, 0, ab2); }
+        const long long atd = matrix(j, Kd, 256, G + c1.w, nullptr, &abd), at2 = matrix(j, 256, 128, G + c2.w, G + c2.b, &ab2);
+        for (int w = 0; w < 2; ++w) { wave(j, w, 1, dirO, dtiles, 0, gout_at(1), 8, 4 * w, atd, Kd, 256, 0, abd); wave(j, 2 + w, 0, act_at(8), 8, 4 * w, gout_at(0), 4, 0, at2, 256, 128, 0, ab2); }
     }
     {
         const int j = new_job(); long long abr, aba;
-        const long long atr = matrix(j, 128, 3, rgb.w, (long long)rgb.b, &abr), ata = matrix(j, 256, 1, alpha.w, (long long)alpha.b, &aba);
-        wave(j, 0, 2, act_at(10), 4, 0, t->dhead, 1, 0, atr, 128, 3, 0, abr);
+        const long long atr = matrix(j, 128, 3, G + rgb.w, G + rgb.b, &abr), ata = matrix(j, 256, 1, G + alpha.w, G + alpha.b, &aba);
+        wave(j, 0, 2, act_at(9), 4, 0, t->dhead, 1, 0, atr, 128, 3, 0, abr);
         for (int w = 0; w < 2; ++w) wave(j, 1 + w, 2, act_at(7), 8, 4 * w, t->dhead, 1, 0, ata, 256, 1, 3, aba);
     }
     n_jobs = (int)jobs.size();
@@ -378,13 +425,17 @@
         ReduceJob &r = reduce.job[reduce.n++];
         const DwJob &j = jobs[rjobs[i].job];
         r.partial = dw_partial + j.first_float + rjobs[i].at; r.n_split = 0; r.stride = j.slot_floats; r.count = rjobs[i].count; r.pair = rjobs[i].pair;
-        r.out = t->grad + rjobs[i].out; r.first = rfirst;
+        r.out = rjobs[i].out; r.first = rfirst;
         rfirst += (rjobs[i].count + 255) / 256 * 256;
         reduce_job.push_back(rjobs[i].job);
     }
 }
 
 void ChainBackend::launch_pack(hipStream_t st) {
+    const float *W = t->w, *w_c1f = W + c1.w + (size_t)t->Kd * 256;
+    FoldArgs f{};
+    f.p[0] = FoldProduct{W + feature.w, 256, 1, w_c1f, 256, 1, fold, nullptr, nullptr, W + feature.b, W + c1.b, fold + FOLD_BIAS, nullptr};
+    hipLaunchKernelGGL(fold_kernel, dim3(8, 9, 1), dim3(256), 0, st, f);
     const PackArgs pa{pack_seg, n_pack, pack_total};
     hipLaunchKernelGGL(pack_kernel, dim3((unsigned)((pack_total + 255) / 256)), dim3(256), 0, st, pa);
 }
@@ -403,7 +454,7 @@
     FwdArgs f = fwd_args(r.M());
     const bool hoist = (t->ipe || r.blur_idx < 0 || r.blur_idx < r.n_geo) && r.S % 32 == 0 && getenv("NERFTEX_TRAIN_NO_DIR_HOIST") == nullptr;
     if (hoist) {
-        DirRowArgs dr{}; dr.r = r; dr.Kd = t->Kd; dr.w = t->w + c1.w; dr.bias = t->w + c1.b; dr.rows = dirrow; dr.splice = t->ipe ? r.blur_idx : -1;
+        DirRowArgs dr{}; dr.r = r; dr.Kd = t->Kd; dr.w = t->w + c1.w; dr.bias = fold + FOLD_BIAS; dr.rows = dirrow; dr.splice = t->ipe ? r.blur_idx : -1;
         hipLaunchKernelGGL(dirrow_kernel, dim3((unsigned)r.n_rays), dim3(256), 0, st, dr);
     }
     f.dirrow = dirrow; f.n_rays = (int)r.n_rays; f.S = r.S;
@@ -457,7 +508,7 @@
     x.out = gout; x.out_stride = gout_stride; x.bits = bits; x.bits_stride = bits_stride;
     launch_dx_chain(st, chain_grid(M), x);
     if (t->pg_mode != 0 || t->ig_mode != 0) {
-        FeatGradArgs p{}; p.dY[0] = gout_at(10); p.W[0] = t->w + trunk[0].w; p.dY[1] = gout_at(5); p.W[1] = t->w + trunk[5].w; p.n_terms = 2;
+        FeatGradArgs p{}; p.dY[0] = gout_at(9); p.W[0] = t->w + trunk[0].w; p.dY[1] = gout_at(4); p.W[1] = t->w + trunk[5].w; p.n_terms = 2;
         p.K = t->Kp; p.ld = ld_pos; p.M = M; p.G = G_pos;
         launch_feat_grad(st, feat_grid(M), ptiles, p);
         FeatGradArgs d{}; d.dY[0] = gout_at(1); d.W[0] = t->w + c1.w; d.n_terms = 1; d.K = t->Kd; d.ld = ld_dir; d.M = M; d.G = G_dir;
@@ -514,6 +565,15 @@
     }
     for (int i = 0; i < rb.n; ++i) rb.job[i].n_split = slots[reduce_job[i]];
     launch_reduce(st, rb);
+    launch_unfold(st);
+}
+void ChainBackend::launch_unfold(hipStream_t st) {
+    const float *W = t->w, *w_c1f = W + c1.w + (size_t)t->Kd * 256, *dwp = dfold, *dbp = dfold + FOLD_BIAS;
+    float *G = t->grad;
+    FoldArgs f{};
+    f.p[0] = FoldProduct{dwp, 256, 1, w_c1f, 1, 256, G + feature.w, nullptr, nullptr, dbp, nullptr, G + feature.b, G + c1.b};
+    f.p[1] = FoldProduct{W + feature.w, 1, 256, dwp, 256, 1, G + c1.w + (size_t)t->Kd * 256, W + feature.b, dbp, nullptr, nullptr, nullptr, nullptr};
+    hipLaunchKernelGGL(fold_kernel, dim3(8, 9, 2), dim3(256), 0, st, f);
 }
 
 void ChainBackend::launch_feat_grad(hipStream_t st, unsigned grid, int tiles, const FeatGradArgs &a) {
@@ -539,12 +599,12 @@
 int ChainBackend::activation(int layer, int64_t n_samples_total, float *out_host) {
     const float *src = nullptr; int tiles = 8;
     if (layer >= 0 && layer < 8) src = act_at(layer);
-    else if (layer == 8) src = act_at(9);
-    else if (layer == 9) { src = act_at(10); tiles = 4; }
+    else if (layer == 8) src = act_at(8);
+    else if (layer == 9) { src = act_at(9); tiles = 4; }
     else if (layer == 10) src = t->sigma;
-    else if (layer >= 20 && layer < 28) src = gout_at(10 - (layer - 20));
+    else if (layer >= 20 && layer < 28) src = gout_at(9 - (layer - 20));
     else if (layer == 28) src = gout_at(1);
-    else if (layer == 29) src = gout_at(2);
+    else if (layer == 29) src = gout_at(1);
     else if (layer == 11) src = t->raw_rgb;
     else if (layer == 30) src = t->dgrad;
     else if ((layer == 40 || layer == 41) && G_pos && ((t->pg_mode != 0 && (t->pg_rows > 0 || t->spg_rays > 0)) || (t->ig_mode != 0 && (t->ig_rays > 0 || t->ig_smp_rays > 0)))) src = layer == 40 ? G_pos : G_dir;
@@ -563,7 +623,16 @@
     }
     const long long nb = (n_samples_total + 31) / 32;
     std::vector<float> tmp((size_t)nb * tiles * 1024);
-    TRAIN_TRY(hipMemcpy(tmp.data(), src, tmp.size() * sizeof(float), hipMemcpyDeviceToHost));
+    const float *from = src;
+    float *dfeat = nullptr;
+    if (layer == 29) {
+        if (t->mem.alloc(&dfeat, tmp.size()) != NTX_OK) return t->mem.rc;
+        hipLaunchKernelGGL(dfeature_kernel, dim3((unsigned)nb), dim3(256), 0, 0, src, t->w + c1.w + (size_t)t->Kd * 256, dfeat);
+        from = dfeat;
+    }
+    const hipError_t copied = hipMemcpy(tmp.data(), from, tmp.size() * sizeof(float), hipMemcpyDeviceToHost);
+    if (dfeat) t->mem.release(dfeat);
+    TRAIN_TRY(copied);
     const int width = tiles * 32;
     for (long long m = 0; m < n_samples_total; ++m)
         for (int row = 0; row < width; ++row) out_host[(size_t)m * width + row] = tmp[o_index(m >> 5, tiles, row, (int)(m & 31))];
@@ -602,7 +671,8 @@
     const long long NB = t->cap_blocks;
     mem.alloc(&c->posO, (size_t)NB * c->ptiles * 1024, true); mem.alloc(&c->dirO, (size_t)NB * c->dtiles * 1024, true);
     c->act_stride = c->gout_stride = NB * 8 * 1024; c->bits_stride = NB * 256;
-    mem.alloc(&c->act, (size_t)c->act_stride * 11); mem.alloc(&c->bits, (size_t)c->bits_stride * 10); mem.alloc(&c->gout, (size_t)c->gout_stride * 11);
+    mem.alloc(&c->act, (size_t)c->act_stride * 10); mem.alloc(&c->bits, (size_t)c->bits_stride * 10); mem.alloc(&c->gout, (size_t)c->gout_stride * 10);
+    mem.alloc(&c->fold, ChainBackend::FOLD_FLOATS, true); mem.alloc(&c->dfold, ChainBackend::FOLD_FLOATS, true);
     mem.alloc(&c->dirrow, (size_t)t->cap_rays * 256);
     c->build_pack();
     c->build_dw_jobs();
diff --git a/nerf_tex_amd/csrc/ntx_train_device.h b/nerf_tex_amd/csrc/ntx_train_device.h
--- a/nerf_tex_amd/csrc/ntx_train_device.h
+++ b/nerf_tex_amd/csrc/ntx_train_device.h
@@ -19,6 +19,12 @@
 TRN_DEV __amdgpu_buffer_rsrc_t make_rsrc(const void *base, long long bytes) {
     const long long b = bytes < 0 ? 0 : (bytes > 0x7ffffff0ll ? 0x7ffffff0ll : bytes);
     return __builtin_amdgcn_make_buffer_rsrc(const_cast<void *>(base), 0, (int)b, 0x00020000);
+}
+
+TRN_DEV void owns_register_file() {
+#if defined(__HIP_DEVICE_COMPILE__)
+    asm volatile("" ::: "a255");
+#endif
 }
 
 TRN_DEV uint32_t o_lane_bytes(int lane) {
@@ -147,10 +153,6 @@
     });
 }
 template <int NMT>
-TRN_DEV void convert_linear(float (&hin)[128], const f32x16 (&prev)[8]) {
-    static_for<NMT * 16>([&](auto V) { constexpr int v = V; hin[v] = prev[v >> 4][v & 15]; });
-}
-template <int NMT>
 TRN_DEV void convert_mask(float (&hin)[128], const f32x16 (&prev)[8], const u32x4 &bits) {
     static_for<NMT * 16>([&](auto V) {
         constexpr int v = V;
@@ -160,7 +162,7 @@
     });
 }
 
-constexpr int AUX_BIAS = 0, AUX_ALPHA_W = 11 * 256, AUX_ALPHA_B = AUX_ALPHA_W + 256, AUX_RGB_W = AUX_ALPHA_B + 4, AUX_RGB_B = AUX_RGB_W + 384,
+constexpr int AUX_BIAS = 0, AUX_ALPHA_W = 10 * 256, AUX_ALPHA_B = AUX_ALPHA_W + 256, AUX_RGB_W = AUX_ALPHA_B + 4, AUX_RGB_B = AUX_RGB_W + 384,
               AUX_FLOATS = AUX_RGB_B + 4;
 template <int MT>
 TRN_DEV void bias_tile(f32x16 (&acc)[8], const float *aux, int layer, int h) {
@@ -187,6 +189,7 @@
 __global__ __launch_bounds__(256) __attribute__((amdgpu_waves_per_eu(1, 1))) void fwd_chain_kernel(FwdArgs a) {
     __shared__ __attribute__((aligned(16))) float aux_lds[AUX_FLOATS];
     __shared__ __attribute__((aligned(16))) float rows_lds[HOIST ? 4 * 256 : 4];
+    owns_register_file();
     ntx::load_aux(aux_lds, a.aux, AUX_FLOATS);
     const int lane = threadIdx.x & 63, n = lane & 31, h = lane >> 5;
     const int wave = __builtin_amdgcn_readfirstlane(blockIdx.x * 4 + (threadIdx.x >> 6)), nwaves = gridDim.x * 4;
@@ -213,7 +216,7 @@
         uint32_t opaque_zero = 0;
         asm volatile("" : "+v"(opaque_zero));
         const float *aux = aux_lds + opaque_zero;
-        const float *rows_aux = rows_lds + opaque_zero + (HOIST ? (threadIdx.x >> 6) * 256 : 0) - AUX_BIAS - 9 * 256;
+        const float *rows_aux = rows_lds + opaque_zero + (HOIST ? (threadIdx.x >> 6) * 256 : 0) - AUX_BIAS - 8 * 256;
         uint32_t sbase = 0;
         f32x16 acc[8];
         float hin[128];
@@ -245,23 +248,20 @@
         auto layer = [&](auto LIc) {
             f32x16 (&cur)[8] = acc; f32x16 (&prev)[8] = acc;
             constexpr int LI = decltype(LIc)::value, in_idx = LI - 1;
-            constexpr bool relu_in = in_idx != 8;
             u32x4 bw = {0u, 0u, 0u, 0u};
-            if constexpr (HOIST && LI == 9) {
+            if constexpr (HOIST && LI == 8) {
                 sbase += (uint32_t)DSG * 8192u;
                 static_for<RING>([&](auto I) { ws.r[I] = wr_load(ws, sbase + (uint32_t)decltype(I)::value * 1024u); });
             }
             static_for<4>([&](auto W) {
                 constexpr int wd = W;
-                if constexpr (relu_in) {
-                    uint32_t w = 0;
-                    static_for<4>([&](auto Q) { convert8_relu_bits<32 * wd + 8 * decltype(Q)::value>(hin, prev, w); });
-                    bw[wd] = w;
-                } else static_for<32>([&](auto V) { constexpr int v = 32 * wd + decltype(V)::value; hin[v] = prev[v >> 4][v & 15]; });
-                const float *bsrc = (HOIST && LI == 9) ? rows_aux : aux;
-                if constexpr (LI < 10 || wd < 2) { bias_tile<2 * wd>(cur, bsrc, LI, h); bias_tile<2 * wd + 1>(cur, bsrc, LI, h); }
+                uint32_t w = 0;
+                static_for<4>([&](auto Q) { convert8_relu_bits<32 * wd + 8 * decltype(Q)::value>(hin, prev, w); });
+                bw[wd] = w;
+                const float *bsrc = (HOIST && LI == 8) ? rows_aux : aux;
+                if constexpr (LI < 9 || wd < 2) { bias_tile<2 * wd>(cur, bsrc, LI, h); bias_tile<2 * wd + 1>(cur, bsrc, LI, h); }
             });
-            if constexpr (relu_in) bits_leave(in_idx < 8 ? in_idx : 8, bw);
+            bits_leave(in_idx, bw);
             if constexpr (LI == 8) {
                 const f32x4 *wa = reinterpret_cast<const f32x4 *>(aux + AUX_ALPHA_W + h * 128);
                 static_for<32>([&](auto I) {
@@ -274,27 +274,27 @@
             __builtin_amdgcn_sched_barrier(0);
             leaves_to(in_idx, 8);
             if constexpr (LI == 5) seg_mem<PSG>(cur, ws, sbase, pb, fetch);
-            if constexpr (LI == 9 && !HOIST) seg_mem<DSG>(cur, ws, sbase, pb, fetch);
+            if constexpr (LI == 8 && !HOIST) seg_mem<DSG>(cur, ws, sbase, pb, fetch);
             if constexpr (LI == 4) rs_in = make_rsrc(a.pos + (size_t)blk * a.ptiles * 1024, (long long)a.ptiles * 4096);
-            if constexpr (LI == 8 && !HOIST) rs_in = make_rsrc(a.dir + (size_t)blk * a.dtiles * 1024, (long long)a.dtiles * 4096);
-            if constexpr (LI == 10) {
+            if constexpr (LI == 7 && !HOIST) rs_in = make_rsrc(a.dir + (size_t)blk * a.dtiles * 1024, (long long)a.dtiles * 4096);
+            if constexpr (LI == 9) {
                 const int nb = blk + nwaves < n_blocks ? blk + nwaves : blk;
                 rs_in = make_rsrc(a.pos + (size_t)nb * a.ptiles * 1024, (long long)a.ptiles * 4096);
             }
             auto extra = [&](auto S, auto MT) {
                 constexpr int s = decltype(S)::value, mt = decltype(MT)::value;
-                if constexpr ((LI == 4 || (LI == 8 && !HOIST) || LI == 10) && mt == 2 && (s == 8 || s == 24)) fetch(std::integral_constant<int, (s == 8 ? 0 : 1)>{});
-                if constexpr (mt == 5 || (LI == 10 && mt == 3)) leave(S);
+                if constexpr ((LI == 4 || (LI == 7 && !HOIST) || LI == 9) && mt == 2 && (s == 8 || s == 24)) fetch(std::integral_constant<int, (s == 8 ? 0 : 1)>{});
+                if constexpr (mt == 5 || (LI == 9 && mt == 3)) leave(S);
             };
-            if constexpr (LI == 10) seg_hidden<128, 4, false>(cur, ws, sbase, hin, extra);
+            if constexpr (LI == 9) seg_hidden<128, 4, false>(cur, ws, sbase, hin, extra);
             else seg_hidden<128, 8, false>(cur, ws, sbase, hin, extra);
         };
-        static_for<10>([&](auto I) { layer(std::integral_constant<int, decltype(I)::value + 1>{}); });
+        static_for<9>([&](auto I) { layer(std::integral_constant<int, decltype(I)::value + 1>{}); });
         {
             u32x4 bw = {0u, 0u, 0u, 0u};
             convert_relu_bits<4>(hin, acc, bw);
             bits_leave(9, bw);
-            leaves_to(10, 4);
+            leaves_to(9, 4);
             static_for<64>([&](auto V) { leave(V); });
             float rgb[3];
             static_for<3>([&](auto C) {
@@ -330,6 +330,7 @@
 
 #ifdef NTX_TRAIN_DX
 __global__ __launch_bounds__(256) __attribute__((amdgpu_waves_per_eu(1, 1))) void dx_chain_kernel(DxArgs a) {
+    owns_register_file();
     const int lane = threadIdx.x & 63, n = lane & 31, h = lane >> 5;
     const int wave = __builtin_amdgcn_readfirstlane(blockIdx.x * 4 + (threadIdx.x >> 6)), nwaves = gridDim.x * 4;
     const int n_blocks = (int)((a.M + 31) >> 5);
@@ -374,13 +375,10 @@
         leaves_to(0, 4);
         seg_hidden<64, 8, true>(acc, ws, sbase, hin, [&](auto S, auto MT) { if constexpr (decltype(MT)::value == 5) leave(S); });
         convert_mask<8>(hin, acc, bw);
-        leaves_to(1, 8);
-        seg_hidden<128, 8, true>(acc, ws, sbase, hin, [&](auto S, auto MT) { if constexpr (decltype(MT)::value == 5) leave(S); });
-        convert_linear<8>(hin, acc);
         static_for<8>([&](auto J) {
             constexpr int j = J;
             bw = fetch_bits(7 - j);
-            leaves_to(2 + j, 8);
+            leaves_to(1 + j, 8);
             seg_hidden<128, 8, true>(acc, ws, sbase, hin, [&](auto S, auto MT) { if constexpr (decltype(MT)::value == 5) leave(S); });
             if constexpr (j == 0) {
                 const float b[1] = {gs};
@@ -388,7 +386,7 @@
             }
             convert_mask<8>(hin, acc, bw);
         });
-        leaves_to(10, 8);
+        leaves_to(9, 8);
         static_for<128>([&](auto V) { leave(V); });
     }
 }
```
